# microsoft/YOLaT-VectorGraphicsRecognition

Measured on AMD Instinct MI355X. Metric: graphs_per_sec, higher is better.
Workload: dtype f32

## Files before the change

### include/yolat_hip.h

```cpp
#ifndef YOLAT_HIP_H
#define YOLAT_HIP_H

#include <stddef.h>
#include <stdint.h>

#ifdef __cplusplus
extern "C" {
#endif

typedef void* yolat_stream_t;

#define YOLAT_E_INVALID   (-1)
#define YOLAT_E_UNSUPPORTED (-2)

#define YOLAT_STATUS_EDGE_RANGE  1
#define YOLAT_STATUS_SEG_UNSORTED 2
#define YOLAT_STATUS_SEG_RANGE   4
#define YOLAT_STATUS_NOT_LOCAL   8


int yolat_abi_version(void);
const char* yolat_strerror(int code);


size_t yolat_csr_work_elems(int64_t N, int64_t E);
int yolat_coo_to_csr(const int64_t* edge, int64_t stride_e, int64_t stride_c, int64_t E, int64_t N,
                     int32_t* row_ptr, int32_t* perm, int32_t* src_csr, int32_t* dst_csr,
                     int32_t* work, int32_t* status, yolat_stream_t stream);

size_t yolat_csc_work_elems(int64_t N);
int yolat_csc_by_source(const int32_t* src_csr, int64_t E, int64_t N, int32_t* col_ptr,
                        int32_t* slots, int32_t* work, yolat_stream_t stream);

int yolat_expand_ranges(const int32_t* start, const int32_t* prefix, int64_t S, int64_t total, int32_t* out,
                        yolat_stream_t stream);
size_t yolat_subgraph_work_elems(int64_t N, int64_t n_sub);
int yolat_subgraph_reindex(const int32_t* node_ids, int64_t n_sub, int64_t N, const int64_t* edge,
                           int64_t stride_e, int64_t stride_c, const int32_t* edge_ids, int64_t m_sub,
                           const int64_t* bbox_idx, int64_t* edge_out, int64_t* bbox_idx_out, int32_t* work,
                           int32_t* status, yolat_stream_t stream);
int yolat_gather_rows_bytes(const void* src, int64_t src_row_bytes, const int32_t* idx, int64_t rows,
                            int64_t row_bytes, void* dst, int64_t dst_row_bytes, yolat_stream_t stream);

int yolat_fixup_offsets(int64_t* edge, int64_t E, const int64_t* edge_ptr, int64_t* bbox_idx, int64_t N,
                        const int64_t* node_ptr, const int64_t* node_off, const int64_t* prop_off, int64_t B,
                        yolat_stream_t stream);

int yolat_segment_ptr(const int64_t* bbox_idx, int64_t N, int64_t P, int32_t* seg_ptr,
                      int32_t* node_seg, int32_t* status, yolat_stream_t stream);

size_t yolat_graph_work_elems(int64_t N, int64_t E);
int yolat_graph_prepare(const int64_t* edge, int64_t stride_e, int64_t stride_c, const float* e_attr,
                        const int64_t* bbox_idx, int64_t E, int64_t N, int64_t P, int32_t* row_ptr,
                        int32_t* perm, int32_t* src_csr, int32_t* dst_csr, float* attr_csr,
                        int32_t* seg_ptr, int32_t* node_seg, int32_t* work, int32_t* status,
                        yolat_stream_t stream);

int yolat_graph_prepare_plan(int64_t N, int64_t E, int64_t other_wgs, int32_t* rows, int32_t* csr_wgs);

int yolat_gather_rows(const float* src, int64_t ld_src, const int32_t* idx, int64_t rows,
                      int64_t width, float* dst, int64_t ld_dst, yolat_stream_t stream);


#define YOLAT_STATS_ROWS 32
size_t yolat_bn_stats_elems(int64_t M, int64_t C);
int yolat_linear_fwd(const float* A, int64_t lda, int64_t M, int64_t K,
                     const float* a_scale, const float* a_shift, int a_relu,
                     const float* W, int64_t ldw, const float* bias, int64_t Nout,
                     const float* o_scale, const float* o_shift, int o_relu,
                     float* Y, int64_t ldy, int accumulate, float* stats, yolat_stream_t stream);

int yolat_linear_sk_x6(const float* A, int64_t lda, int64_t M, int64_t K, const float* W, int64_t ldw, const float* bias,
                       int64_t Nout, const float* o_scale, const float* o_shift, int o_relu, float* Y, int64_t ldy,
                       yolat_stream_t stream);

int yolat_linear_segmax_fwd(const float* A, int64_t lda, int64_t M, int64_t K, const float* W,
                            int64_t ldw, const float* bias, int64_t Nout, const float* o_scale,
                            const float* o_shift, const int32_t* node_seg, float* pool, int64_t ldpool,
                            yolat_stream_t stream);

int yolat_linear_fwd_wt(const float* A, int64_t lda, int64_t M, int64_t K,
                        const float* Wt, int64_t ldw, int64_t Nout,
                        float* Y, int64_t ldy, int accumulate, yolat_stream_t stream);

size_t yolat_linear_bwd_w_work_elems(int64_t M, int64_t Nout, int64_t K);
int yolat_linear_bwd_w(const float* dY, int64_t lddy, int64_t M, int64_t Nout,
                       const float* A, int64_t lda, int64_t K,
                       const float* a_scale, const float* a_shift, int a_relu,
                       float* dW, int64_t lddw, float* db, int accumulate,
                       float* partial, yolat_stream_t stream);

int yolat_bn_finalize(const float* stats, int64_t M, int64_t C, const float* gamma,
                      const float* beta, float* running_mean, float* running_var,
                      float momentum, float eps, float* save_mean, float* save_invstd,
                      float* scale, float* shift, yolat_stream_t stream);

int yolat_bn_eval_coeffs(const float* gamma, const float* beta, const float* running_mean,
                         const float* running_var, float eps, int64_t C, float* scale,
                         float* shift, yolat_stream_t stream);

int yolat_scale_shift_relu(const float* Y, int64_t ldy, int64_t M, int64_t C, const float* scale,
                           const float* shift, int relu, float* Z, int64_t ldz,
                           yolat_stream_t stream);

size_t yolat_bn_bwd_work_elems(int64_t M, int64_t C);
int yolat_bn_relu_bwd(const float* dZ, int64_t lddz, const float* Y, int64_t ldy, int64_t M,
                      int64_t C, const float* gamma, const float* save_mean,
                      const float* save_invstd, const float* scale, const float* shift, int relu,
                      float* dgamma, float* dbeta, int accumulate, float* dY, int64_t lddy,
                      float* work, yolat_stream_t stream);


int yolat_edge_lin1_fwd(const float* x, int64_t ldx, int64_t N, int64_t Cin,
                        const int32_t* src_csr, const int32_t* dst_csr, const float* attr_csr,
                        int64_t E, const float* W1, int64_t ldw, const float* b1, int64_t C,
                        const float* o_scale, const float* o_shift, int o_relu,
                        float* H1, int64_t ldh, float* stats, yolat_stream_t stream);

int yolat_edge_lin1_bwd_w(const float* dH1, int64_t lddh, int64_t E, int64_t C,
                          const float* x, int64_t ldx, int64_t N, int64_t Cin,
                          const int32_t* src_csr, const int32_t* dst_csr, const float* attr_csr,
                          float* dW1, int64_t lddw, float* db1, int accumulate, float* partial,
                          yolat_stream_t stream);

int yolat_edge_lin1_bwd_x(const float* dH1, int64_t lddh, int64_t E, int64_t C, const float* W1,
                          int64_t ldw, int64_t Cin, float* dG, int64_t lddg,
                          yolat_stream_t stream);

int yolat_edge_scatter_bwd(const float* dG, int64_t lddg, int64_t Cin, const int32_t* row_ptr,
                           const int32_t* col_ptr, const int32_t* slots, int64_t N, float* dX,
                           int64_t lddx, int accumulate, yolat_stream_t stream);

int yolat_edge_mlp2_eval(const float* x, int64_t ldx, int64_t N, int64_t Cin, const int32_t* src_csr,
                         const int32_t* dst_csr, const float* attr_csr, int64_t E, const float* W1,
                         const float* b1, const float* s1, const float* t1, const float* W2,
                         const float* b2, const float* s2, const float* t2, int64_t C, float* H2,
                         int64_t ldh, yolat_stream_t stream);

int yolat_graph_prepare_node_uv(const int64_t* edge, int64_t stride_e, int64_t stride_c, const float* e_attr,
                                const int64_t* bbox_idx, int64_t E, int64_t N, int64_t P, int32_t* row_ptr,
                                int32_t* perm, int32_t* src_csr, int32_t* dst_csr, float* attr_csr,
                                int32_t* seg_ptr, int32_t* node_seg, int32_t* work, int32_t* status, const float* x,
                                int64_t ldx, int64_t Cin, const float* Wuv, const float* uv_bias, const float* Wr,
                                const float* br,
                                const float* Wn, const float* bn, const float* sn, const float* tn, int64_t C,
                                float* UV, int64_t ld_uv, float* f_out, int64_t ld_fo, float* s_out, int64_t ld_so,
                                yolat_stream_t stream);

int yolat_conv_split_w1(const float* W1, int64_t Cin, int64_t C, float* Wuv, float* Wc4, yolat_stream_t stream);
int yolat_node_uv_eval(const float* f_in, int64_t ld_f, const float* s_in, int64_t ld_s, int64_t N, int64_t Cin,
                       const float* Wuv, const float* uv_bias, const float* Wr, const float* br, const float* Wn,
                       const float* bn, const float* sn, const float* tn, int64_t C, float* UV, int64_t ld_uv,
                       float* f_out, int64_t ld_fo, float* s_out, int64_t ld_so, yolat_stream_t stream);
int yolat_edge_uv_lin1_fwd(const float* UV, int64_t ld_uv, const int32_t* src_csr, const int32_t* dst_csr,
                           const float* attr_csr, int64_t E, const float* Wc4, const float* b1, int64_t C,
                           float* H1, int64_t ldh, float* stats, yolat_stream_t stream);

int yolat_edge_uv_sums(const float* dH1, int64_t ldh, const int32_t* row_ptr, const int32_t* col_ptr,
                       const int32_t* slots, int64_t N, int64_t C, float* dUV, int64_t ld_uv, yolat_stream_t stream);
int yolat_conv_merge_dw1(const float* dWuv, const float* dWc4, int64_t Cin, int64_t C, float* dW1, int64_t lddw,
                         int accumulate, yolat_stream_t stream);

#define YOLAT_EDGE_AUTO 0
#define YOLAT_EDGE_TILES 1
#define YOLAT_EDGE_WS_F32 2
#define YOLAT_EDGE_WS_X6 3
int yolat_edge_uv_mlp2_mean_eval(const float* UV, int64_t ld_uv, const int32_t* src_csr, const int32_t* dst_csr,
                                 const float* attr_csr, const int32_t* row_ptr, int64_t N, int64_t E,
                                 const float* Wc4, const float* b1, const float* s1, const float* t1,
                                 const float* W2, const float* b2, const float* s2, const float* t2, int64_t C,
                                 float* f_out, int64_t ld_fo, yolat_stream_t stream);
int yolat_edge_uv_mlp2_mean_eval_variant(const float* UV, int64_t ld_uv, const int32_t* src_csr,
                                         const int32_t* dst_csr, const float* attr_csr, const int32_t* row_ptr,
                                         int64_t N, int64_t E, const float* Wc4, const float* b1, const float* s1,
                                         const float* t1, const float* W2, const float* b2, const float* s2,
                                         const float* t2, int64_t C, float* f_out, int64_t ld_fo, int variant,
                                         yolat_stream_t stream);
int yolat_edge_uv_mlp2_eval(const float* UV, int64_t ld_uv, const int32_t* src_csr, const int32_t* dst_csr,
                            const float* attr_csr, int64_t E, const float* Wc4, const float* b1, const float* s1,
                            const float* t1, const float* W2, const float* b2, const float* s2, const float* t2,
                            int64_t C, float* H2, int64_t ldh, yolat_stream_t stream);

int yolat_node_side_eval(const float* f_in, int64_t ld_f, const float* s_in, int64_t ld_s, int64_t N,
                         int64_t Cin, const float* Wr, const float* br, const float* Wn, const float* bn,
                         const float* sn, const float* tn, const float* H2, int64_t ldh,
                         const int32_t* row_ptr, int64_t E, int64_t C, float* f_out, int64_t ld_fo,
                         float* s_out, int64_t ld_so, yolat_stream_t stream);

int yolat_csr_mean_fwd(const float* H, int64_t ldh, int64_t C, const float* h_scale,
                       const float* h_shift, int h_relu, const int32_t* row_ptr, int64_t N,
                       float* out, int64_t ldo, int accumulate, yolat_stream_t stream);

int yolat_csr_mean_bwd(const float* dOut, int64_t lddo, int64_t C, const int32_t* row_ptr,
                       const int32_t* dst_csr, int64_t E, float* dM, int64_t lddm,
                       yolat_stream_t stream);

int yolat_segment_mean_fwd(const float* X, int64_t ldx, int64_t D, const float* x_scale,
                           const float* x_shift, int x_relu, const int32_t* seg_ptr, int64_t P,
                           float* Y, int64_t ldy, yolat_stream_t stream);
int yolat_segment_max_fwd(const float* X, int64_t ldx, int64_t D, const float* x_scale,
                          const float* x_shift, int x_relu, const int32_t* seg_ptr, int64_t P,
                          int64_t N, float* Y, int64_t ldy, int32_t* arg ,
                          yolat_stream_t stream);
int yolat_fusion_pair_eval(const float* A, int64_t lda, int64_t N, int64_t D, const float* Wf, const float* bf,
                           const float* sf, const float* tf, int64_t F, const int32_t* node_seg, float* pool,
                           int64_t ldpool, const float* S, int64_t lds, int64_t P, const float* Wfs,
                           const float* bfs, const float* sfs, const float* tfs, float* Ys, int64_t ldys,
                           yolat_stream_t stream);

int yolat_pool_prepare(const float* feats, const float* fsup, int64_t ld, int64_t D, int64_t F,
                       const int32_t* seg_ptr, int64_t P, float* Z, int64_t ldz, yolat_stream_t stream);

int yolat_segment_mean_bwd(const float* dY, int64_t lddy, int64_t D, const int32_t* seg_ptr,
                           const int32_t* node_seg, int64_t N, float* dX, int64_t lddx,
                           yolat_stream_t stream);
int yolat_segment_max_bwd(const float* dY, int64_t lddy, int64_t D, const int32_t* arg,
                          const int32_t* node_seg, int64_t N, float* dX, int64_t lddx,
                          yolat_stream_t stream);

size_t yolat_fusion_pool_train_saved_elems(int64_t K, int64_t F, int64_t P);
size_t yolat_fusion_pool_train_work_elems(int64_t N, int64_t K, int64_t F, int64_t P);
int yolat_fusion_pool_train_fwd(const float* A, int64_t lda, int64_t N, int64_t K, const float* W,
                                const float* bias, int64_t F, const float* gamma, const float* beta,
                                float* running_mean, float* running_var, float momentum, float eps,
                                const int32_t* node_seg, int64_t P, float* Z, int64_t ldz, float* coef,
                                float* saved, float* work, yolat_stream_t stream);
int yolat_fusion_pool_train_bwd(const float* A, int64_t lda, int64_t N, int64_t K, const float* W,
                                const float* gamma, int64_t F, const float* coef, const float* saved,
                                const int32_t* node_seg, const int32_t* seg_ptr, int64_t P, const float* gZ,
                                int64_t ldg, float* dW, float* dbias, float* dgamma, float* dbeta, float* dA,
                                int64_t ldda, float* work, yolat_stream_t stream);
#define YOLAT_FUS_BWD_COLS 1
#define YOLAT_FUS_BWD_DW 2
#define YOLAT_FUS_BWD_DA 4
#define YOLAT_FUS_BWD_ALL 7
int yolat_fusion_pool_train_bwd_parts(const float* A, int64_t lda, int64_t N, int64_t K, const float* W,
                                      const float* gamma, int64_t F, const float* coef, const float* saved,
                                      const int32_t* node_seg, const int32_t* seg_ptr, int64_t P, const float* gZ,
                                      int64_t ldg, float* dW, float* dbias, float* dgamma, float* dbeta, float* dA,
                                      int64_t ldda, float* work, int parts, yolat_stream_t stream);


size_t yolat_softmax_ce_work_elems(int64_t P);
int yolat_softmax_ce(const float* logits, int64_t ld, const int64_t* labels, int64_t P, int64_t K,
                     float* loss, float* dlogits, int64_t lddl, float* work, yolat_stream_t stream);

int yolat_sigmoid(const float* z, int64_t ldz, int64_t P, int64_t K, float* out, int64_t ldo, yolat_stream_t stream);
int yolat_sigmoid_bwd(const float* dp, int64_t lddp, const float* p, int64_t ldp, int64_t P, int64_t K, float* dz,
                      int64_t lddz, yolat_stream_t stream);
size_t yolat_bce_work_elems(int64_t P);
int yolat_bce(const float* prob, int64_t ld, const int64_t* labels, int64_t P, int64_t K, float* loss, float* dprob,
              int64_t lddp, float* work, yolat_stream_t stream);
int yolat_sigmoid_bce(const float* logits, int64_t ld, const int64_t* labels, int64_t P, int64_t K, float* loss,
                      float* dlogits, int64_t lddl, float* prob, int64_t ldp, float* work, yolat_stream_t stream);

int yolat_adam_step(float* param, const float* grad, float* exp_avg, float* exp_avg_sq, int64_t n,
                    float lr, float beta1, float beta2, float eps, float weight_decay,
                    int64_t step, float grad_scale, yolat_stream_t stream);

#define YOLAT_MAX_LAYERS 8

typedef struct {
  int64_t Cin;
  const float *W1, *b1, *s1, *t1;
  const float *W2, *b2, *s2, *t2;
  const float *Wr, *br;
  const float *Wn, *bn, *sn, *tn;
  const float *Wuv, *Wc4;
  const float *Wuvf, *uvb, *Wc4f, *t2f;
  const uint16_t *Wfr_x6[3];
  const float *tfr;
  const uint16_t *Wn_x6[3];
  const float *tn_fold;
  const float *Wnx, *tnx;
} yolat_conv_eval;

#define YOLAT_CLS_X6_MAX_ROWS 2048
#define YOLAT_CLS1_X6_MIN_ROWS 1024
#define YOLAT_NODE_X6_MIN_ROWS 65536
typedef struct {
  int32_t n_blocks, n_blocks_out, n_classes, reserved;
  int64_t C;
  int64_t F;
  int64_t H1, H2;
  yolat_conv_eval conv[YOLAT_MAX_LAYERS];
  const float *Wf, *bf, *sf, *tf;
  const uint16_t *Wf_hi, *Wf_mid, *Wf_lo;
  const float *tf_fold;
  const uint16_t *Wfs_hi, *Wfs_mid, *Wfs_lo;
  const float *tfs_fold;
  const float *Wfs, *bfs, *sfs, *tfs;
  const float *Wc1, *bc1, *sc1, *tc1;
  const float *Wc2, *bc2, *sc2, *tc2;
  const float *Wc3, *bc3;
  const uint16_t *Wc_x6[3];
  const float *tc_fold[3];
  const uint16_t *Wc1_gx;
  const float *tc1_gx;
} yolat_model_eval;

size_t yolat_forward_eval_workspace_bytes(const yolat_model_eval* m, int64_t N, int64_t E, int64_t P);

int yolat_forward_eval(const yolat_model_eval* m, const float* x, int64_t ldx, const int64_t* edge,
                       int64_t stride_e, int64_t stride_c, const float* e_attr,
                       const int64_t* bbox_idx, int64_t N, int64_t E, int64_t P, float* logits,
                       int64_t ld_logits, void* workspace, size_t workspace_bytes, int32_t* status,
                       yolat_stream_t stream);
int yolat_forward_eval_primed(const yolat_model_eval* m, const float* x, int64_t ldx, const int64_t* edge,
                              int64_t stride_e, int64_t stride_c, const float* e_attr,
                              const int64_t* bbox_idx, int64_t N, int64_t E, int64_t P, float* logits,
                              int64_t ld_logits, void* workspace, size_t workspace_bytes, int32_t* status,
                              yolat_stream_t stream);

typedef struct { const void* ptr; int64_t bytes; } yolat_span;
int yolat_collate_pack(void* dst, const int64_t* field_off, const yolat_span* spans, int64_t n_fields, int64_t n_items);
int yolat_item_csr_host(const int64_t* edge, int64_t stride_e, int64_t stride_c, const float* e_attr,
                        const int64_t* bbox_idx, int64_t E, int64_t N, int64_t P, int32_t* row_ptr, int32_t* perm,
                        int32_t* src, int32_t* dst, float* attr, int32_t* seg_ptr, int32_t* node_seg, int32_t* status);
typedef struct {
  int64_t N, E, P;
  const int32_t *row_ptr, *src, *dst;
  const float* attr;
  const int32_t *seg_ptr, *node_seg;
} yolat_item_csr;
int yolat_collate_csr_pack(const yolat_item_csr* items, int64_t B, int32_t* row_ptr, int32_t* src, int32_t* dst,
                           float* attr, int32_t* seg_ptr, int32_t* node_seg);

#define YOLAT_MAX_KEYS 8
typedef struct {
  int64_t n_keys;
  yolat_span key[YOLAT_MAX_KEYS];
  int64_t rows[YOLAT_MAX_KEYS];
  yolat_item_csr csr;
  int32_t fix[YOLAT_MAX_KEYS];
  int32_t node_key, prop_key;
} yolat_item_desc;
int yolat_collate_batch(const yolat_item_desc* const* items, int64_t B, void* dst, int64_t cap, int64_t* off,
                        int64_t* total, int64_t* slices, int64_t* totals);

typedef struct yolat_loader yolat_loader;
typedef struct {
  void* device;
  int64_t total, n_keys, B, N, E, P;
  int64_t off[YOLAT_MAX_KEYS + 6];
  const int64_t* slices;
  int32_t slot, rc;
} yolat_loader_batch;
yolat_loader* yolat_loader_create(int slots);
int yolat_loader_submit(yolat_loader* loader, const yolat_item_desc* const* items, int64_t B);
int yolat_loader_next(yolat_loader* loader, yolat_stream_t consumer_stream, yolat_loader_batch* out);
int yolat_loader_release(yolat_loader* loader, int slot, yolat_stream_t consumer_stream);
void yolat_loader_destroy(yolat_loader* loader);

typedef struct {
  const int32_t *row_ptr, *src, *dst;
  const float* attr;
  const int32_t *seg_ptr, *node_seg;
} yolat_graph_csr;
int yolat_forward_eval_csr(const yolat_model_eval* m, const float* x, int64_t ldx, const yolat_graph_csr* g, int64_t N,
                           int64_t E, int64_t P, float* logits, int64_t ld_logits, void* workspace,
                           size_t workspace_bytes, yolat_stream_t stream);

typedef struct {
  const yolat_model_eval* base;
  const uint16_t* Wuv[YOLAT_MAX_LAYERS];
  const uint16_t* Wr[YOLAT_MAX_LAYERS];
  const uint16_t* Wn[YOLAT_MAX_LAYERS];
  const uint16_t* W2[YOLAT_MAX_LAYERS];
  const float* uv_scale[YOLAT_MAX_LAYERS];
  const float* uv_shift[YOLAT_MAX_LAYERS];
  const uint16_t *Wf, *Wfs, *Wc1, *Wc2, *Wc3;
  const float* t2f[YOLAT_MAX_LAYERS];
  const uint16_t *Wf_fold, *Wfs_fold;
  const float *tf_fold, *tfs_fold;
  const void* conv_local;
} yolat_model_eval_bf16;

size_t yolat_conv_local_pack_bytes(int64_t n_layers);
int yolat_conv_local_pack(const yolat_model_eval_bf16* m, void* dst, size_t dst_bytes, yolat_stream_t stream);
void yolat_conv_local_tune(int nw, int g0, int abl, long long* stamps);
int yolat_conv_stack_local_bf16(const yolat_model_eval_bf16* m, const void* pack, const float* x, int64_t ldx,
                                const yolat_graph_csr* g, int64_t N, int64_t E, int64_t P, uint16_t* feats,
                                int64_t ld_feats, float* Z, int64_t ldz, int32_t* flag, yolat_stream_t stream);

#define YOLAT_LOC_UNGROUPED 1
#define YOLAT_LOC_CROSSING  2
#define YOLAT_LOC_MALFORMED 4
typedef struct yolat_locality {
  int32_t known, flags, max_nodes, max_edges;
} yolat_locality;
size_t yolat_batch_locality_workspace_bytes(int64_t N, int64_t E, int64_t P);
int yolat_batch_locality(const int64_t* edge, int64_t stride_e, int64_t stride_c, const int64_t* bbox_idx, int64_t N,
                         int64_t E, int64_t P, int32_t* info, void* workspace, size_t workspace_bytes,
                         yolat_stream_t stream);
int yolat_conv_local_fits(const yolat_locality* loc, int64_t P);
// ... 248 lines not shown
```

### yolat_vectorgraphicsrecognition_amd/_lib.py

```python
import ctypes
import os

_HERE = os.path.dirname(os.path.abspath(__file__))
LIB_PATH = os.environ.get("YOLAT_LIB_PATH") or os.path.join(_HERE, "libyolat_hip.so")

c_p = ctypes.c_void_p
c_i64 = ctypes.c_int64
c_int = ctypes.c_int
c_f = ctypes.c_float
c_sz = ctypes.c_size_t

YOLAT_MAX_LAYERS = 8


class ConvEval(ctypes.Structure):
    _fields_ = ([("Cin", c_i64)] + [(n, c_p) for n in
                                    ("W1", "b1", "s1", "t1", "W2", "b2", "s2", "t2", "Wr", "br", "Wn", "bn", "sn", "tn",
                                     "Wuv", "Wc4", "Wuvf", "uvb", "Wc4f", "t2f")] +
                [("Wfr_x6", c_p * 3), ("tfr", c_p), ("Wn_x6", c_p * 3), ("tn_fold", c_p), ("Wnx", c_p), ("tnx", c_p)])


class ModelEval(ctypes.Structure):
    _fields_ = ([("n_blocks", ctypes.c_int32), ("n_blocks_out", ctypes.c_int32), ("n_classes", ctypes.c_int32),
                 ("reserved", ctypes.c_int32), ("C", c_i64), ("F", c_i64), ("H1", c_i64), ("H2", c_i64),
# ... 42 lines not shown


class Locality(ctypes.Structure):
    _fields_ = [("known", ctypes.c_int32), ("flags", ctypes.c_int32), ("max_nodes", ctypes.c_int32),
                ("max_edges", ctypes.c_int32)]


class TrainLin(ctypes.Structure):
    _fields_ = [("W", c_p), ("b", c_p)]


class TrainBn(ctypes.Structure):
    _fields_ = [("gamma", c_p), ("beta", c_p), ("running_mean", c_p), ("running_var", c_p), ("num_batches_tracked", c_p),
                ("momentum", c_f), ("eps", c_f)]


class TrainConv(ctypes.Structure):
    _fields_ = [("Cin", c_i64), ("nn0", TrainLin), ("bn1", TrainBn), ("nn3", TrainLin), ("bn4", TrainBn), ("lin_r", TrainLin),
                ("node", TrainLin), ("bn_node", TrainBn)]


class TrainModel(ctypes.Structure):
    _fields_ = [("n_blocks", ctypes.c_int32), ("n_blocks_out", ctypes.c_int32), ("n_classes", ctypes.c_int32),
                ("half", ctypes.c_int32), ("C", c_i64), ("F", c_i64), ("H1", c_i64), ("H2", c_i64),
                ("conv", TrainConv * YOLAT_MAX_LAYERS), ("fus", TrainLin), ("fus_bn", TrainBn), ("fus_s", TrainLin),
                ("fus_s_bn", TrainBn), ("c1", TrainLin), ("c1_bn", TrainBn), ("c2", TrainLin), ("c2_bn", TrainBn),
                ("c3", TrainLin), ("param_base", c_p), ("grad_base", c_p)]


class AdamArgs(ctypes.Structure):
    _fields_ = [("exp_avg", c_p), ("exp_avg_sq", c_p), ("n", c_i64), ("step", c_i64), ("lr", c_f), ("beta1", c_f),
                ("beta2", c_f), ("eps", c_f), ("weight_decay", c_f), ("grad_scale", c_f)]


class PredictTree(ctypes.Structure):
    _fields_ = [("R", c_i64), ("Ctot", c_i64), ("B", c_i64), ("root_row", c_p), ("root_range", c_p), ("child_ptr", c_p),
                ("child_row", c_p), ("child_range", c_p), ("image_root_ptr", c_p)]


class GraphCsr(ctypes.Structure):
    _fields_ = [("row_ptr", c_p), ("src", c_p), ("dst", c_p), ("attr", c_p), ("seg_ptr", c_p), ("node_seg", c_p)]


SIGNATURES = {
    "yolat_abi_version": (c_int, []),
    "yolat_strerror": (ctypes.c_char_p, [c_int]),
    "yolat_csr_work_elems": (c_sz, [c_i64, c_i64]),
    "yolat_coo_to_csr": (c_int, [c_p, c_i64, c_i64, c_i64, c_i64, c_p, c_p, c_p, c_p, c_p, c_p, c_p]),
    "yolat_edge_mlp2_eval": (c_int, [c_p, c_i64, c_i64, c_i64, c_p, c_p, c_p, c_i64, c_p, c_p, c_p, c_p, c_p, c_p, c_p,
                                      c_p, c_i64, c_p, c_i64, c_p]),
    "yolat_node_side_eval": (c_int, [c_p, c_i64, c_p, c_i64, c_i64, c_i64, c_p, c_p, c_p, c_p, c_p, c_p, c_p, c_i64,
                                      c_p, c_i64, c_i64, c_p, c_i64, c_p, c_i64, c_p]),
    "yolat_fusion_pool_train_saved_elems": (c_sz, [c_i64, c_i64, c_i64]),
    "yolat_fusion_pool_train_work_elems": (c_sz, [c_i64, c_i64, c_i64, c_i64]),
    "yolat_fusion_pool_train_fwd": (c_int, [c_p, c_i64, c_i64, c_i64, c_p, c_p, c_i64, c_p, c_p, c_p, c_p, c_f, c_f,
                                             c_p, c_i64, c_p, c_i64, c_p, c_p, c_p, c_p]),
    "yolat_fusion_pool_train_bwd": (c_int, [c_p, c_i64, c_i64, c_i64, c_p, c_p, c_i64, c_p, c_p, c_p, c_p, c_i64, c_p,
                                             c_i64, c_p, c_p, c_p, c_p, c_p, c_i64, c_p, c_p]),
    "yolat_fusion_pool_train_bwd_parts": (c_int, [c_p, c_i64, c_i64, c_i64, c_p, c_p, c_i64, c_p, c_p, c_p, c_p, c_i64, c_p,
                                                   c_i64, c_p, c_p, c_p, c_p, c_p, c_i64, c_p, c_int, c_p]),
    "yolat_fusion_pool_train_fwd_bf16": (c_int, [c_p, c_i64, c_i64, c_i64, c_p, c_p, c_i64, c_p, c_p, c_p, c_p, c_f, c_f,
                                                  c_p, c_i64, c_p, c_i64, c_p, c_p, c_p, c_p]),
    "yolat_fusion_pool_train_bwd_parts_bf16": (c_int, [c_p, c_i64, c_i64, c_i64, c_p, c_p, c_i64, c_p, c_p, c_p, c_p, c_i64,
                                                        c_p, c_i64, c_p, c_p, c_p, c_p, c_p, c_i64, c_p, c_int, c_p]),
    "yolat_bt_linear_fwd": (c_int, [c_p, c_i64, c_i64, c_i64, c_p, c_p, c_int, c_p, c_i64, c_p, c_i64, c_p, c_i64, c_p, c_p]),
    "yolat_bt_linear_fwd_wt": (c_int, [c_p, c_i64, c_i64, c_i64, c_p, c_i64, c_i64, c_p, c_i64, c_int, c_p]),
    "yolat_bt_linear_bwd_w_work_elems": (c_sz, [c_i64, c_i64, c_i64]),
    "yolat_bt_linear_bwd_w": (c_int, [c_p, c_i64, c_i64, c_i64, c_p, c_i64, c_i64, c_p, c_p, c_int, c_p, c_i64, c_p, c_p,
                                       c_p]),
    "yolat_expand_ranges": (c_int, [c_p, c_p, c_i64, c_i64, c_p, c_p]),
    "yolat_subgraph_work_elems": (c_sz, [c_i64, c_i64]),
    "yolat_subgraph_reindex": (c_int, [c_p, c_i64, c_i64, c_p, c_i64, c_i64, c_p, c_i64, c_p, c_p, c_p, c_p, c_p, c_p]),
    "yolat_gather_rows_bytes": (c_int, [c_p, c_i64, c_p, c_i64, c_i64, c_p, c_i64, c_p]),
    "yolat_fixup_offsets": (c_int, [c_p, c_i64, c_p, c_p, c_i64, c_p, c_p, c_p, c_i64, c_p]),
    "yolat_conv_split_w1": (c_int, [c_p, c_i64, c_i64, c_p, c_p, c_p]),
    "yolat_node_uv_eval": (c_int, [c_p, c_i64, c_p, c_i64, c_i64, c_i64, c_p, c_p, c_p, c_p, c_p, c_p, c_p, c_p, c_i64,
                                    c_p, c_i64, c_p, c_i64, c_p, c_i64, c_p]),
    "yolat_edge_uv_mlp2_eval": (c_int, [c_p, c_i64, c_p, c_p, c_p, c_i64, c_p, c_p, c_p, c_p, c_p, c_p, c_p, c_p, c_i64,
                                         c_p, c_i64, c_p]),
    "yolat_edge_uv_mlp2_mean_eval": (c_int, [c_p, c_i64, c_p, c_p, c_p, c_p, c_i64, c_i64, c_p, c_p, c_p, c_p, c_p, c_p,
                                              c_p, c_p, c_i64, c_p, c_i64, c_p]),
    "yolat_edge_uv_mlp2_mean_eval_variant": (c_int, [c_p, c_i64, c_p, c_p, c_p, c_p, c_i64, c_i64, c_p, c_p, c_p, c_p,
                                                      c_p, c_p, c_p, c_p, c_i64, c_p, c_i64, c_int, c_p]),
    "yolat_edge_uv_sums": (c_int, [c_p, c_i64, c_p, c_p, c_p, c_i64, c_i64, c_p, c_i64, c_p]),
    "yolat_conv_merge_dw1": (c_int, [c_p, c_p, c_i64, c_i64, c_p, c_i64, c_int, c_p]),
    "yolat_fusion_pair_eval": (c_int, [c_p, c_i64, c_i64, c_i64, c_p, c_p, c_p, c_p, c_i64, c_p, c_p, c_i64, c_p, c_i64,
                                        c_i64, c_p, c_p, c_p, c_p, c_p, c_i64, c_p]),
    "yolat_graph_prepare_node_uv": (c_int, [c_p, c_i64, c_i64, c_p, c_p, c_i64, c_i64, c_i64] + [c_p] * 9 +
                                    [c_p, c_i64, c_i64] + [c_p] * 8 + [c_i64, c_p, c_i64, c_p, c_i64, c_p, c_i64, c_p]),
    "yolat_csc_work_elems": (c_sz, [c_i64]),
    "yolat_csc_by_source": (c_int, [c_p, c_i64, c_i64, c_p, c_p, c_p, c_p]),
    "yolat_segment_ptr": (c_int, [c_p, c_i64, c_i64, c_p, c_p, c_p, c_p]),
    "yolat_graph_work_elems": (c_sz, [c_i64, c_i64]),
    "yolat_graph_prepare": (c_int, [c_p, c_i64, c_i64, c_p, c_p, c_i64, c_i64, c_i64, c_p, c_p, c_p, c_p, c_p,
                                    c_p, c_p, c_p, c_p, c_p]),
    "yolat_graph_prepare_plan": (c_int, [c_i64, c_i64, c_i64, c_p, c_p]),
    "yolat_gather_rows": (c_int, [c_p, c_i64, c_p, c_i64, c_i64, c_p, c_i64, c_p]),
    "yolat_bn_stats_elems": (c_sz, [c_i64, c_i64]),
    "yolat_linear_fwd": (c_int, [c_p, c_i64, c_i64, c_i64, c_p, c_p, c_int,
                                 c_p, c_i64, c_p, c_i64, c_p, c_p, c_int,
                                 c_p, c_i64, c_int, c_p, c_p]),
    "yolat_linear_sk_x6": (c_int, [c_p, c_i64, c_i64, c_i64, c_p, c_i64, c_p, c_i64, c_p, c_p, c_int, c_p, c_i64, c_p]),
    "yolat_linear_segmax_fwd": (c_int, [c_p, c_i64, c_i64, c_i64, c_p, c_i64, c_p, c_i64, c_p, c_p, c_p, c_p, c_i64,
                                        c_p]),
    "yolat_linear_fwd_wt": (c_int, [c_p, c_i64, c_i64, c_i64, c_p, c_i64, c_i64, c_p, c_i64, c_int, c_p]),
    "yolat_linear_bwd_w_work_elems": (c_sz, [c_i64, c_i64, c_i64]),
    "yolat_linear_bwd_w": (c_int, [c_p, c_i64, c_i64, c_i64, c_p, c_i64, c_i64, c_p, c_p, c_int,
                                   c_p, c_i64, c_p, c_int, c_p, c_p]),
    "yolat_bn_finalize": (c_int, [c_p, c_i64, c_i64, c_p, c_p, c_p, c_p, c_f, c_f, c_p, c_p, c_p, c_p, c_p]),
    "yolat_bn_eval_coeffs": (c_int, [c_p, c_p, c_p, c_p, c_f, c_i64, c_p, c_p, c_p]),
    "yolat_scale_shift_relu": (c_int, [c_p, c_i64, c_i64, c_i64, c_p, c_p, c_int, c_p, c_i64, c_p]),
    "yolat_bn_bwd_work_elems": (c_sz, [c_i64, c_i64]),
    "yolat_bn_relu_bwd": (c_int, [c_p, c_i64, c_p, c_i64, c_i64, c_i64, c_p, c_p, c_p, c_p, c_p, c_int,
                                  c_p, c_p, c_int, c_p, c_i64, c_p, c_p]),
    "yolat_edge_lin1_fwd": (c_int, [c_p, c_i64, c_i64, c_i64, c_p, c_p, c_p, c_i64, c_p, c_i64, c_p,
                                    c_i64, c_p, c_p, c_int, c_p, c_i64, c_p, c_p]),
    "yolat_edge_lin1_bwd_w": (c_int, [c_p, c_i64, c_i64, c_i64, c_p, c_i64, c_i64, c_i64, c_p, c_p, c_p,
                                      c_p, c_i64, c_p, c_int, c_p, c_p]),
    "yolat_edge_lin1_bwd_x": (c_int, [c_p, c_i64, c_i64, c_i64, c_p, c_i64, c_i64, c_p, c_i64, c_p]),
    "yolat_edge_scatter_bwd": (c_int, [c_p, c_i64, c_i64, c_p, c_p, c_p, c_i64, c_p, c_i64, c_int, c_p]),
    "yolat_csr_mean_fwd": (c_int, [c_p, c_i64, c_i64, c_p, c_p, c_int, c_p, c_i64, c_p, c_i64, c_int, c_p]),
    "yolat_csr_mean_bwd": (c_int, [c_p, c_i64, c_i64, c_p, c_p, c_i64, c_p, c_i64, c_p]),
    "yolat_segment_mean_fwd": (c_int, [c_p, c_i64, c_i64, c_p, c_p, c_int, c_p, c_i64, c_p, c_i64, c_p]),
    "yolat_segment_max_fwd": (c_int, [c_p, c_i64, c_i64, c_p, c_p, c_int, c_p, c_i64, c_i64, c_p, c_i64,
                                      c_p, c_p]),
    "yolat_pool_prepare": (c_int, [c_p, c_p, c_i64, c_i64, c_i64, c_p, c_i64, c_p, c_i64, c_p]),
    "yolat_segment_mean_bwd": (c_int, [c_p, c_i64, c_i64, c_p, c_p, c_i64, c_p, c_i64, c_p]),
    "yolat_segment_max_bwd": (c_int, [c_p, c_i64, c_i64, c_p, c_p, c_i64, c_p, c_i64, c_p]),
    "yolat_softmax_ce_work_elems": (c_sz, [c_i64]),
    "yolat_softmax_ce": (c_int, [c_p, c_i64, c_p, c_i64, c_i64, c_p, c_p, c_i64, c_p, c_p]),
    "yolat_sigmoid": (c_int, [c_p, c_i64, c_i64, c_i64, c_p, c_i64, c_p]),
    "yolat_sigmoid_bwd": (c_int, [c_p, c_i64, c_p, c_i64, c_i64, c_i64, c_p, c_i64, c_p]),
    "yolat_bce_work_elems": (c_sz, [c_i64]),
    "yolat_bce": (c_int, [c_p, c_i64, c_p, c_i64, c_i64, c_p, c_p, c_i64, c_p, c_p]),
    "yolat_sigmoid_bce": (c_int, [c_p, c_i64, c_p, c_i64, c_i64, c_p, c_p, c_i64, c_p, c_i64, c_p, c_p]),
    "yolat_adam_step": (c_int, [c_p, c_p, c_p, c_p, c_i64, c_f, c_f, c_f, c_f, c_f, c_i64, c_f, c_p]),
    "yolat_profile_enabled": (c_int, []),
    "yolat_profile_enable": (c_int, [c_int]),
    "yolat_profile_reset": (c_int, []),
    "yolat_profile_count": (c_int, []),
    "yolat_profile_get": (c_int, [c_int, ctypes.c_char_p, c_int, ctypes.POINTER(c_f), ctypes.POINTER(c_int),
                                  ctypes.POINTER(ctypes.c_double), ctypes.POINTER(ctypes.c_double)]),
    "yolat_forward_eval_workspace_bytes": (c_sz, [ctypes.POINTER(ModelEval), c_i64, c_i64, c_i64]),
    "yolat_forward_eval": (c_int, [ctypes.POINTER(ModelEval), c_p, c_i64, c_p, c_i64, c_i64, c_p, c_p, c_i64, c_i64,
                                   c_i64, c_p, c_i64, c_p, c_sz, c_p, c_p]),
    "yolat_forward_eval_primed": (c_int, [ctypes.POINTER(ModelEval), c_p, c_i64, c_p, c_i64, c_i64, c_p, c_p, c_i64,
                                          c_i64, c_i64, c_p, c_i64, c_p, c_sz, c_p, c_p]),
    "yolat_edge_uv_lin1_fwd": (c_int, [c_p, c_i64, c_p, c_p, c_p, c_i64, c_p, c_p, c_i64, c_p, c_i64, c_p, c_p]),
    "yolat_nms_work_bytes": (c_sz, [c_i64]),
    "yolat_nms": (c_int, [c_p, c_p, c_i64, c_f, c_p, c_p, c_p, c_sz, c_p]),
    "yolat_detect_scores": (c_int, [c_p, c_i64, c_i64, c_i64, c_p, c_p, c_i64, c_p, c_int, c_p, c_p]),
    "yolat_nms_batched_work_bytes": (c_sz, [c_i64, c_i64, c_i64]),
    "yolat_nms_batched": (c_int, [c_p, c_i64, c_i64, c_p, c_i64, c_f, c_f, c_int, c_p, c_p, c_p, c_sz, c_p]),
    "yolat_detect_match": (c_int, [c_p, c_p, c_i64, c_p, c_p, c_i64, c_p, c_p, c_i64, c_p, c_p]),
    "yolat_f32_to_bf16": (c_int, [c_p, c_i64, c_p, c_p]),
    "yolat_edge_uv_lin1_fwd_h": (c_int, [c_p, c_i64, c_p, c_p, c_p, c_i64, c_p, c_p, c_i64, c_p, c_i64, c_p, c_p]),
    "yolat_linear_fwd_h": (c_int, [c_p, c_i64, c_i64, c_i64, c_p, c_p, c_int, c_p, c_i64, c_p, c_i64, c_p, c_i64, c_p,
                                   c_p, c_p]),
    "yolat_csr_mean_fwd_h": (c_int, [c_p, c_i64, c_i64, c_p, c_p, c_int, c_p, c_i64, c_p, c_i64, c_int, c_p]),
    "yolat_csr_mean_bwd_h": (c_int, [c_p, c_i64, c_i64, c_p, c_p, c_i64, c_p, c_i64, c_p]),
    "yolat_bn_relu_bwd_h": (c_int, [c_p, c_i64, c_p, c_i64, c_i64, c_i64, c_p, c_p, c_p, c_p, c_int, c_p, c_p, c_int,
                                    c_p, c_i64, c_p, c_p]),
    "yolat_linear_bwd_w_h": (c_int, [c_p, c_i64, c_i64, c_i64, c_p, c_int, c_i64, c_i64, c_p, c_p, c_int, c_p, c_i64,
                                     c_p, c_int, c_p, c_p]),
    "yolat_linear_fwd_wt_h": (c_int, [c_p, c_i64, c_i64, c_i64, c_p, c_i64, c_i64, c_p, c_i64, c_p, c_p]),
    "yolat_edge_uv_sums_h": (c_int, [c_p, c_i64, c_p, c_p, c_p, c_i64, c_i64, c_p, c_i64, c_p]),
    "yolat_split_bf16x3": (c_int, [c_p, c_i64, c_i64, c_i64, c_p, c_p, c_p, c_p, c_p]),
    "yolat_linear_fwd_rows_x6": (c_int, [c_p, c_i64, c_i64, c_i64, c_p, c_p, c_int, c_p, c_i64, c_p, c_i64, c_p, c_i64, c_p,
                                         c_p, c_p]),
    "yolat_node_uv_eval_x6": (c_int, [c_p, c_i64, c_p, c_i64, c_i64, c_p, c_p, c_p, c_p, c_p, c_p, c_p, c_p, c_p, c_i64,
                                      c_p, c_i64, c_p, c_i64, c_p]),
    "yolat_fusion_pair_eval_x6": (c_int, [c_p, c_i64, c_i64, c_i64, c_p, c_p, c_p, c_p, c_i64, c_p, c_p, c_i64, c_p,
                                          c_i64, c_i64, c_p, c_p, c_p, c_p, c_p, c_i64, c_p]),
    "yolat_inv_degree": (c_int, [c_p, c_i64, c_p, c_p]),
    "yolat_bn_csr_work_elems": (c_sz, [c_i64, c_i64]),
    "yolat_bn_csr_bwd_stats": (c_int, [ctypes.POINTER(BnCsrGrad), c_i64, c_i64, c_p, c_p, c_int, c_p, c_p, c_p]),
    "yolat_linear_bwd_w_csr": (c_int, [ctypes.POINTER(BnCsrGrad), c_i64, c_i64, c_p, c_i64, c_i64, c_p, c_p, c_int, c_p,
                                       c_i64, c_p, c_int, c_p, c_p]),
    "yolat_linear_fwd_wt_csr": (c_int, [ctypes.POINTER(BnCsrGrad), c_i64, c_i64, c_p, c_i64, c_i64, c_p, c_i64, c_p]),
# ... 107 lines not shown
```

### yolat_vectorgraphicsrecognition_amd/csrc/common.hpp

```cpp
#pragma once
#include <hip/hip_runtime.h>
#include <stdint.h>

#include "../../include/yolat_hip.h"

typedef float f32x16 __attribute__((ext_vector_type(16)));
typedef float f32x4 __attribute__((ext_vector_type(4)));

#define YL_LAUNCH_CHECK()                          \
  do {                                             \
    hipError_t e__ = hipGetLastError();            \
    if (e__ != hipSuccess) return (int)e__;        \
  } while (0)

#define YL_TRY(call)            \
  do {                          \
    int rc__ = (call);          \
    if (rc__ != 0) return rc__; \
  } while (0)

static inline int yl_cdiv(long a, long b) { return (int)((a + b - 1) / b); }
static inline bool yl_aligned16(const void* p) { return (((uintptr_t)p) & 15) == 0; }

struct Carver {
// ... 694 lines not shown
#pragma unroll
        for (int k = 0; k < N3_KMAX; ++k) acc = fmaf(x[k], w[j][k], acc);
        v[j] = fmaxf(fmaf(acc + b[j], sc[j], sh[j]), floor);
      }
      const int row = rb + u;
      if (row < r1) {
        if (Yh != nullptr) {
          uint2 o;
          o.x = yl_pack_bf16(v[0], v[1]); o.y = yl_pack_bf16(v[2], v[3]);
          *reinterpret_cast<uint2*>(Yh + (long)row * ldy + col) = o;
        } else {
          *reinterpret_cast<float4*>(Y + (long)row * ldy + col) = make_float4(v[0], v[1], v[2], v[3]);
        }
      }
    }
  }
}

bool yl_node3_smallk_ok(const NodeUv& a);
bool yl_node3_smallk_shape_ok(const NodeUv& a);
int yl_node3_smallk(const NodeUv& a, hipStream_t st, YlGate gate = YlGate{nullptr, 0});
int yl_fusion_rows_x6_key64(const float* A, long lda, long N, long K, const float* W, const float* bias, long F,
                            const float* sgn, const int* node_seg, unsigned long long* keys, uint16_t* wsplit,
                            yolat_stream_t stream);
int yl_fusion_rows_bf16_key64(const float* A, long lda, long N, long K, const float* W, const float* bias, long F,
                              const float* sgn, const int* node_seg, unsigned long long* keys, uint16_t* wimg,
                              yolat_stream_t stream);
#define YL_POOL_ZERO 1
#define YL_POOL_MAX 2
#define YL_POOL_MEAN 4
struct PoolRider {
  const float* feats; const float* fsup; long ld; int D, F, P; const int* seg_ptr; float* Z; long ldz;
  int parts, blocks;
};
__device__ __forceinline__ void yl_pool_rider(const PoolRider& r, int vb, int nvb, int tid, int nthreads) {
  const int wz = (r.parts & YL_POOL_ZERO) ? r.F : 0, wx = (r.parts & YL_POOL_MAX) ? r.D : 0,
            wm = (r.parts & YL_POOL_MEAN) ? r.D : 0;
  const int W = wz + wx + wm;
  const long total = (long)r.P * W;
  for (long i = (long)vb * nthreads + tid; i < total; i += (long)nvb * nthreads) {
    const int p = (int)(i / W), c = (int)(i - (long)p * W);
    float* z = r.Z + (long)p * r.ldz;
    if (c < wz) { z[c] = 0.f; continue; }
    const bool is_max = c < wz + wx;
    const int k = is_max ? c - wz : c - wz - wx;
    const float* src = (is_max ? r.feats : r.fsup) + k;
    const int r0 = r.seg_ptr[p], r1 = r.seg_ptr[p + 1];
    float best = 0.f, sm = 0.f;
    bool any = false;
    int q = r0;
    for (; q + 8 <= r1; q += 8) {
      float v[8];
#pragma unroll
      for (int j = 0; j < 8; ++j) v[j] = src[(long)(q + j) * r.ld];
#pragma unroll
      for (int j = 0; j < 8; ++j) {
        if (!any || v[j] > best) { best = v[j]; any = true; }
        sm += v[j];
      }
    }
    for (; q < r1; ++q) {
      const float v = src[(long)q * r.ld];
      if (!any || v > best) { best = v; any = true; }
      sm += v;
    }
    if (is_max) z[r.F + k] = best;
    else {
      const int cnt = r1 - r0;
      z[2 * r.F + r.D + k] = sm / (float)(cnt > 1 ? cnt : 1);
    }
  }
}
struct EdgeNext {
  const float* Wp; const float* bias; float* UV; long ld_uv; float* root; long ld_root;
  const float* s_in; long ld_si; const float* Wn; const float* bn; const float* sn; const float* tn;
  float* s_out; long ld_so; int s_tiles;
};
int yl_edge_tile_groups(int64_t N, int64_t E);
int yl_edge_uv_mlp2_mean_eval_impl(const float* UV, int64_t ld_uv, const int32_t* src_csr, const int32_t* dst_csr,
                                   const float* attr_csr, const int32_t* row_ptr, int64_t N, int64_t E, const float* Wc4,
                                   const float* b1, const float* s1, const float* t1, const float* W2, const float* b2,
                                   const float* s2, const float* t2, int64_t C, float* f_out, int64_t ld_fo, int variant,
                                   const PoolRider* rider, int* rode, const EdgeNext* next, int* did_next,
                                   yolat_stream_t stream);
int yl_fusion_pair_eval_x6_impl(const float* A, int64_t lda, int64_t N, int64_t D, const uint16_t* Wh, const uint16_t* Wm,
                                const uint16_t* Wl, const float* tfold, int64_t F, const int32_t* node_seg, float* pool,
                                int64_t ldpool, const float* S, int64_t lds, int64_t P, const uint16_t* Wsh,
                                const uint16_t* Wsm, const uint16_t* Wsl, const float* tsfold, float* Ys, int64_t ldys,
                                const PoolRider* rider, yolat_stream_t stream);
int yl_pool_prepare_parts(const float* feats, const float* fsup, int64_t ld, int64_t D, int64_t F, const int32_t* seg_ptr,
                          int64_t P, float* Z, int64_t ldz, int parts, yolat_stream_t stream);
bool yl_profile_on();
void yl_stage_begin(const char* name, double flops, double bytes, yolat_stream_t stream);
void yl_stage_end(yolat_stream_t stream);

struct YlLocalIn {
  const int32_t *row_ptr, *src, *dst; const float* attr; const int32_t* seg_ptr;
  const int64_t* edge; int64_t se, sc; const int32_t* eptr;
  int32_t* status;
};
int yl_local_prep(const int64_t* edge, int64_t se, int64_t sc, const int64_t* bbox_idx, int64_t N, int64_t E, int64_t P,
                  int32_t* seg_ptr, int32_t* node_seg, int32_t* eptr, int32_t* status, int32_t* info, bool vouched,
                  hipStream_t st);

int yl_graph_prepare_impl(const int64_t* edge, int64_t stride_e, int64_t stride_c, const float* e_attr,
                          const int64_t* bbox_idx, int64_t E, int64_t N, int64_t P, int32_t* row_ptr, int32_t* perm,
                          int32_t* src_csr, int32_t* dst_csr, float* attr_csr, int32_t* seg_ptr, int32_t* node_seg,
                          int32_t* work, int32_t* status, const NodeUv* extra, bool primed, yolat_stream_t stream);
template <int BK>
__device__ __forceinline__ void node_uv_tile(const NodeUv& a, int x, int y) {
  if (y < 2) gemm_nt_tile<64, 64, BK, DenseOp, DenseOp, false>(a.af, a.wuv, a.euv, a.N, 2 * a.C, a.Cin, x, y);
  else if (y == 2) gemm_nt_tile<64, 64, BK, DenseOp, DenseOp, false>(a.af, a.wr, a.er, a.N, a.C, a.Cin, x, 0);
  else gemm_nt_tile<64, 64, BK, DenseOp, DenseOp, false>(a.as, a.wn, a.en, a.N, a.C, a.Cin, x, 0);
}

template <int BK>
__global__ void __launch_bounds__(256) k_gemm_nt_node3(NodeUv a) {
  node_uv_tile<BK>(a, blockIdx.x, blockIdx.y);
}

template <class AL, class BL, bool B_NFAST>
__global__ void __launch_bounds__(256) k_gemm_nt_sk(AL A, BL B, Epilogue ep, int M, int N, int K) {
  constexpr int BT = 32, BK = 128, LD = BK + 1;
  __shared__ float smem[2 * BT * LD];
  float* As = smem;
  float* Bs = smem + BT * LD;
  const int tid = threadIdx.x, wave = tid >> 6, lane = tid & 63;
  const int l31 = lane & 31, lhi = lane >> 5;
  int rt_, ct_;
  yl_xcd_tile(rt_, ct_);
  const int row0 = rt_ * BT, col0 = ct_ * BT;
  const bool fastA = A.vec != 0, fastB = B.vec != 0;
  auto map_r = [](int i) { return 4 * ((i >> 5) & 7) + ((i & 31) >> 3); };
  auto map_q = [](int i) { return 8 * (i >> 8) + (i & 7); };
  const EpiPre pre = epi_prefetch(ep, row0, col0 + l31, M, N);

  f32x16 acc;
#pragma unroll
  for (int r = 0; r < 16; ++r) acc[r] = 0.f;

  float ra0[4][4], rb0[4][4], ra1[4][4], rb1[4][4];
  auto fetch = [&](int k0, float (&ra)[4][4], float (&rb)[4][4]) {
    const bool full = (k0 + BK <= K);
    if (full && fastA) {
#pragma unroll
      for (int t = 0; t < 4; ++t) {
        const int i = tid + t * 256;
        A.template load4<true>(row0 + map_r(i), k0 + 4 * map_q(i), ra[t]);
      }
    } else {
#pragma unroll
      for (int t = 0; t < 4; ++t) {
        const int i = tid + t * 256;
        A.template load4<false>(row0 + map_r(i), k0 + 4 * map_q(i), ra[t]);
      }
    }
    if (full && fastB) {
#pragma unroll
      for (int t = 0; t < 4; ++t) {
        const int i = tid + t * 256;
        const int n = B_NFAST ? (i % BT) : map_r(i);
        const int kq = B_NFAST ? (i / BT) : map_q(i);
        B.template load4<true>(col0 + n, k0 + 4 * kq, rb[t]);
      }
    } else {
#pragma unroll
      for (int t = 0; t < 4; ++t) {
        const int i = tid + t * 256;
        const int n = B_NFAST ? (i % BT) : map_r(i);
        const int kq = B_NFAST ? (i / BT) : map_q(i);
        B.template load4<false>(col0 + n, k0 + 4 * kq, rb[t]);
      }
    }
  };
  auto stage = [&](float (&ra)[4][4], float (&rb)[4][4]) {
#pragma unroll
    for (int t = 0; t < 4; ++t) {
      const int i = tid + t * 256;
      float* d = As + map_r(i) * LD + 4 * map_q(i);
      d[0] = ra[t][0]; d[1] = ra[t][1]; d[2] = ra[t][2]; d[3] = ra[t][3];
      const int n = B_NFAST ? (i % BT) : map_r(i);
      const int kq = B_NFAST ? (i / BT) : map_q(i);
      float* e = Bs + n * LD + 4 * kq;
      e[0] = rb[t][0]; e[1] = rb[t][1]; e[2] = rb[t][2]; e[3] = rb[t][3];
    }
  };
  auto compute = [&]() {
    const int kb = wave * 32;
#pragma unroll
    for (int kk = 0; kk < 32; kk += 2) {
      const float a = As[l31 * LD + kb + kk + lhi];
// ... 321 lines not shown
```

### yolat_vectorgraphicsrecognition_amd/csrc/edge.hip

```cpp
#include "common.hpp"
#include <stdlib.h>

extern "C" int yolat_edge_lin1_fwd(const float* x, int64_t ldx, int64_t N, int64_t Cin,
                                   const int32_t* src_csr, const int32_t* dst_csr,
                                   const float* attr_csr, int64_t E, const float* W1, int64_t ldw,
                                   const float* b1, int64_t C, const float* o_scale,
                                   const float* o_shift, int o_relu, float* H1, int64_t ldh,
                                   float* stats, yolat_stream_t stream) {
  if (E < 0 || N <= 0 || Cin <= 0 || C <= 0 || !x || !W1) return YOLAT_E_INVALID;
  if (E == 0) return 0;
  if (!src_csr || !dst_csr || !attr_csr || !H1 || E >= (1LL << 31)) return YOLAT_E_INVALID;
  const long K = 2 * Cin + 4;
  if (ldw < K || ldh < C || ldx < Cin) return YOLAT_E_INVALID;
  if ((o_scale == nullptr) != (o_shift == nullptr)) return YOLAT_E_INVALID;
  EdgeOp a = yl_edge(x, ldx, Cin, src_csr, dst_csr, attr_csr, E);
  DenseOp b = yl_dense(W1, ldw, C, K);
  Epilogue ep;
  ep.bias = b1; ep.scale = o_scale; ep.shift = o_shift; ep.relu = o_relu;
  ep.Y = H1; ep.ldy = ldh; ep.accumulate = 0; ep.stats = stats; ep.seg = nullptr; ep.pool = nullptr; ep.ldpool = 0;
  hipStream_t st = (hipStream_t)stream;
  dim3 grid(yl_cdiv(E, 64), yl_cdiv(C, 64));
  if (K <= 16)
    hipLaunchKernelGGL((k_gemm_nt<64, 64, 16, EdgeOp, DenseOp, false>), grid, dim3(256), 0, st, a,
                       b, ep, (int)E, (int)C, (int)K);
// ... 361 lines not shown
#pragma unroll 8
    for (int kk = 0; kk < 64; kk += 2) {
      const float av = Hs[(wm * 32 + l31) * LDH + kk + lhi];
      const float bv = W2s[(wn * 32 + l31) * LDH + kk + lhi];
      acc2 = __builtin_amdgcn_mfma_f32_32x32x2f32(av, bv, acc2, 0, 0, 0);
    }
    if (c0 == e0) EDGE_STAMP(5);
    __syncthreads();
#pragma unroll
    for (int r = 0; r < 16; ++r) {
      const int row = wm * 32 + (r & 3) + 8 * (r >> 2) + 4 * lhi;
      Hs[row * LDH + col] = fmaxf(fmaf(acc2[r] + bias2, sc2, sh2), 0.f);
    }
    __syncthreads();
    if (c0 == e0) EDGE_STAMP(6);
#pragma unroll
    for (int j = 0; j < NG; ++j) {
      if (rb + 16 * j < nn) {
        const int lo = my_b[j] > c0 ? my_b[j] : c0;
        const int hi = my_e[j] < c0 + 64 ? my_e[j] : c0 + 64;
        for (int e = lo; e < hi; ++e) {
          const float* m = Hs + (e - c0) * LDH + 4 * q;
          sum[j].x += m[0]; sum[j].y += m[1]; sum[j].z += m[2]; sum[j].w += m[3];
        }
      }
    }
    if (c0 == e0) EDGE_STAMP(7);
    __syncthreads();
  }
  EDGE_STAMP(8);
#pragma unroll
  for (int j = 0; j < NG; ++j) {
    const int deg = my_e[j] - my_b[j];
    if (rb + 16 * j < nn && deg > 0) {
      const float inv = 1.f / (float)deg;
      float4* o = reinterpret_cast<float4*>(f_out + (long)(n0 + rb + 16 * j) * ld_fo + 4 * q);
      float4 d = fo[j];
      d.x = yl_mul_rn(sum[j].x, inv) + d.x; d.y = yl_mul_rn(sum[j].y, inv) + d.y;
      d.z = yl_mul_rn(sum[j].z, inv) + d.z; d.w = yl_mul_rn(sum[j].w, inv) + d.w;
      *o = d;
      fo[j] = d;
    }
  }
  EDGE_STAMP(9);
  if constexpr (NG == 1 && NEXT) {
    float bfa[16], bfb[16];
#pragma unroll
    for (int ks = 0; ks < 16; ++ks) bfa[ks] = nx.Wp[(wave * 16 + ks) * 64 + lane];
    float* frow = Hs + rb * LDH + 4 * q;
    const float4 fz = (rb < nn) ? fo[0] : make_float4(0.f, 0.f, 0.f, 0.f);
    frow[0] = fz.x; frow[1] = fz.y; frow[2] = fz.z; frow[3] = fz.w;
    __syncthreads();
    const int fr = lane & 15, fk = lane >> 4;
#pragma unroll
    for (int t = 0; t < 3; ++t) {
      const int ct = wave + 4 * t;
      if (t < 2) {
#pragma unroll
        for (int ks = 0; ks < 16; ++ks) bfb[ks] = nx.Wp[((ct + 4) * 16 + ks) * 64 + lane];
      }
      const int col = ct * 16 + fr;
      const float bias = nx.bias[col];
      f32x4 acc = {0.f, 0.f, 0.f, 0.f};
#pragma unroll
      for (int ks = 0; ks < 16; ++ks)
        acc = __builtin_amdgcn_mfma_f32_16x16x4f32(Hs[fr * LDH + 4 * ks + fk], bfa[ks], acc, 0, 0, 0);
#pragma unroll
      for (int r = 0; r < 4; ++r) {
        const int row = 4 * fk + r;
        if (row < nn) {
          const float v = acc[r] + bias;
          if (col < 128) nx.UV[(long)(n0 + row) * nx.ld_uv + col] = v;
          else nx.root[(long)(n0 + row) * nx.ld_root + (col - 128)] = v;
        }
      }
#pragma unroll
      for (int ks = 0; ks < 16; ++ks) bfa[ks] = bfb[ks];
    }
  }
  EDGE_STAMP(10);
#ifdef YOLAT_EDGE_STAMPS
  if (threadIdx.x == 0 && blockIdx.x < 4096) edge_stamps_d[nx.Wp != nullptr ? 0 : 1][blockIdx.x * 16 + 11] = (long long)((e1g - e0g + 63) / 64);
#endif
}

typedef __bf16 yl_bf16x8 __attribute__((ext_vector_type(8)));
typedef unsigned yl_u32x4 __attribute__((ext_vector_type(4)));
__device__ __forceinline__ void yl_split8(const float x[8], yl_bf16x8& h, yl_bf16x8& m, yl_bf16x8& l) {
  yl_u32x4 ph, pm, pl;
#pragma unroll
  for (int i = 0; i < 4; ++i) {
    const unsigned x0 = __float_as_uint(x[2 * i]), x1 = __float_as_uint(x[2 * i + 1]);
    const yl_f32x2 xv = {x[2 * i], x[2 * i + 1]};
    const yl_f32x2 hv = {__uint_as_float(x0 & 0xffff0000u), __uint_as_float(x1 & 0xffff0000u)};
    const yl_f32x2 hmv = {__uint_as_float(x0 & 0xffffff00u), __uint_as_float(x1 & 0xffffff00u)};
    const yl_f32x2 mv = hmv - hv, lv = xv - hmv;
    ph[i] = __builtin_amdgcn_perm(x1, x0, 0x07060302u);
    pm[i] = __builtin_amdgcn_perm(__float_as_uint(mv.y), __float_as_uint(mv.x), 0x07060302u);
    pl[i] = __builtin_amdgcn_perm(__float_as_uint(lv.y), __float_as_uint(lv.x), 0x07060302u);
  }
  h = *reinterpret_cast<yl_bf16x8*>(&ph);
  m = *reinterpret_cast<yl_bf16x8*>(&pm);
  l = *reinterpret_cast<yl_bf16x8*>(&pl);
}

template <bool FOLD, bool X6>
__global__ void __launch_bounds__(512, 4) k_edge_uv_mlp2_mean_ws(const float* __restrict__ UV, long ld_uv,
                                                                 const int* __restrict__ src,
                                                                 const int* __restrict__ dst,
                                                                 const float* __restrict__ attr,
                                                                 const int* __restrict__ row_ptr, int N, int E, int chunk,
                                                                 const float* __restrict__ Wc4,
                                                                 const float* __restrict__ b1,
                                                                 const float* __restrict__ s1,
                                                                 const float* __restrict__ t1,
                                                                 const float* __restrict__ W2,
                                                                 const float* __restrict__ b2,
                                                                 const float* __restrict__ s2,
                                                                 const float* __restrict__ t2, float* f_out, long ld_fo) {
  constexpr int LDH = 68, TILE = 64 * LDH;
  __shared__ __attribute__((aligned(16))) float Hs[2 * TILE];
  __shared__ __attribute__((aligned(16))) float Ms[2 * TILE];
  __shared__ int seg_start[2][66];
  __shared__ int seg_node[2][64];
  __shared__ int seg_info[2][4];
  __shared__ __attribute__((aligned(16))) float carry_s[2][64];
  __shared__ int carry_cnt_s[2];
  const int tid = threadIdx.x, wave = tid >> 6, lane = tid & 63;
  const long c_lo = (long)blockIdx.x * chunk;
  if (c_lo >= E) return;
  const long c_hi = c_lo + chunk;
  int eS = 0, eE = E;
  if (c_lo > 0) {
    const int n = dst[c_lo];
    eS = (row_ptr[n] == (int)c_lo) ? (int)c_lo : row_ptr[n + 1];
  }
  if (c_hi < E) {
    const int n = dst[c_hi];
    eE = (row_ptr[n] == (int)c_hi) ? (int)c_hi : row_ptr[n + 1];
  }
  if (eS >= eE) return;
  const int np = (eE - eS + 63) >> 6;

  if (wave >= 4) {
    const int cw = wave - 4, wm = cw >> 1, wn = cw & 1, l31 = lane & 31, lhi = lane >> 5;
    const int col = wn * 32 + l31;
    const float bias2 = (!FOLD && b2) ? b2[col] : 0.f, sc2 = s2 ? s2[col] : 1.f, sh2 = s2 ? t2[col] : 0.f;
    auto store_messages = [&](const f32x16& acc, int p) {
      float* ms = Ms + (p & 1) * TILE;
#pragma unroll
      for (int r = 0; r < 16; ++r) {
        const int row = wm * 32 + (r & 3) + 8 * (r >> 2) + 4 * lhi;
        ms[row * LDH + col] = FOLD ? fmaxf(fmaf(acc[r], sc2, sh2), 0.f) : fmaxf(fmaf(acc[r] + bias2, sc2, sh2), 0.f);
      }
    };
    if (X6) {
      yl_bf16x8 Bh[4], Bm[4], Bl[4];
#pragma unroll
      for (int ks = 0; ks < 4; ++ks) {
        const float4* wp = reinterpret_cast<const float4*>(W2 + (long)col * 64 + 16 * ks + 8 * lhi);
        const float4 w0 = wp[0], w1 = wp[1];
        float x[8] = {w0.x, w0.y, w0.z, w0.w, w1.x, w1.y, w1.z, w1.w};
        if (FOLD) {
#pragma unroll
          for (int i = 0; i < 8; ++i) x[i] *= sc2;
        }
// ... 142 lines not shown
    }
    const int first_next = __shfl(dm_nxt, 0);
    if (lane == 63) seg_info[bsel][2] = (c0 + 64 < eE && first_next == dm_cur) ? 1 : 0;
    prev_last = __shfl(dm_cur, 63);
    dm_cur = dm_nxt;
    dm_nxt = dst[yl_min(c0 + 128 + lane, eE - 1)];
  };
  float4 fo0 = make_float4(0.f, 0.f, 0.f, 0.f);
  auto fo_load = [&](int P) {
    const int bsel = P & 1;
    const int k = yl_min(rb, seg_info[bsel][0] - 1);
    fo0 = *reinterpret_cast<const float4*>(f_out + (long)seg_node[bsel][k] * ld_fo + 4 * q);
  };
  auto aggregate = [&](int P) {
    const int bsel = P & 1;
    const float* ms = Ms + bsel * TILE + 4 * q;
    const int nseg = seg_info[bsel][0], cont_in = seg_info[bsel][1], cont_out = seg_info[bsel][2];
    for (int k = rb; k < nseg; k += 16) {
      const int lo = seg_start[bsel][k], hi = seg_start[bsel][k + 1];
      float4 sm = make_float4(0.f, 0.f, 0.f, 0.f);
      int cn = 0;
      if (k == 0 && cont_in) {
        sm = *reinterpret_cast<const float4*>(&carry_s[bsel ^ 1][4 * q]);
        cn = carry_cnt_s[bsel ^ 1];
      }
      for (int r = lo; r < hi; ++r) {
        const float4 m = *reinterpret_cast<const float4*>(ms + r * LDH);
        sm.x += m.x; sm.y += m.y; sm.z += m.z; sm.w += m.w;
      }
      cn += hi - lo;
      if (k == nseg - 1 && cont_out) {
        *reinterpret_cast<float4*>(&carry_s[bsel][4 * q]) = sm;
        if (q == 0) carry_cnt_s[bsel] = cn;
      } else {
        const float inv = 1.f / (float)cn;
        float4* o = reinterpret_cast<float4*>(f_out + (long)seg_node[bsel][k] * ld_fo + 4 * q);
        float4 d = fo0;
        if (k != rb) d = *o;
        d.x = yl_mul_rn(sm.x, inv) + d.x; d.y = yl_mul_rn(sm.y, inv) + d.y;
        d.z = yl_mul_rn(sm.z, inv) + d.z; d.w = yl_mul_rn(sm.w, inv) + d.w;
        *o = d;
      }
    }
  };
  load_idx(eS);
  gather(eS);
  load_idx(eS + 64);
  layer1(Hs);
  gather(eS + 64);
  load_idx(eS + 128);
  __syncthreads();
  for (int p = 0; p < np; ++p) {
    layer1(Hs + ((p + 1) & 1) * TILE);
    gather(eS + 64 * (p + 2));
    load_idx(eS + 64 * (p + 3));
    meta(p);
    if (p >= 1) aggregate(p - 1);
    fo_load(p);
    __syncthreads();
  }
  aggregate(np - 1);
}

static long edge_tile_npt(long N, long E) {
  long npt = (56 * N) / E;
  const long npt2 = (112 * N) / E < 16 ? (112 * N) / E : 16;
  if (npt2 >= 2 * npt - 2 && N / (npt2 > 0 ? npt2 : 1) >= 8192) npt = npt2;
  if (npt < 1) npt = 1;
  if (npt > 64) npt = 64;
  return npt;
}
int yl_edge_tile_groups(int64_t N, int64_t E) {
  if (N <= 0 || E <= 0) return 0;
  const int variant = E >= 131072 ? (yl_strict_fp32() ? YOLAT_EDGE_WS_F32 : YOLAT_EDGE_WS_X6) : YOLAT_EDGE_TILES;
  if (variant != YOLAT_EDGE_TILES) return 0;
  return edge_tile_npt(N, E) <= 16 ? 1 : 4;
}

int yl_edge_uv_mlp2_mean_eval_impl(const float* UV, int64_t ld_uv, const int32_t* src_csr, const int32_t* dst_csr,
                                   const float* attr_csr, const int32_t* row_ptr, int64_t N, int64_t E, const float* Wc4,
                                   const float* b1, const float* s1, const float* t1, const float* W2, const float* b2,
                                   const float* s2, const float* t2, int64_t C, float* f_out, int64_t ld_fo, int variant,
                                   const PoolRider* rider, int* rode, const EdgeNext* next, int* did_next,
                                   yolat_stream_t stream) {
  if (rode) *rode = 0;
  if (did_next) *did_next = 0;
  if (E < 0 || N <= 0 || !UV || !Wc4 || !W2 || !row_ptr || !f_out) return YOLAT_E_INVALID;
  if (variant < YOLAT_EDGE_AUTO || variant > YOLAT_EDGE_WS_X6) return YOLAT_E_INVALID;
  if (C != 64) return YOLAT_E_UNSUPPORTED;
  if (E == 0) return 0;
  if (!src_csr || !dst_csr || !attr_csr || E >= (1LL << 31) || ld_fo < C || ld_uv < 2 * C) return YOLAT_E_INVALID;
  if ((s1 == nullptr) != (t1 == nullptr) || (s2 == nullptr) != (t2 == nullptr)) return YOLAT_E_INVALID;
  if (ld_uv % 4 != 0 || ld_fo % 4 != 0 || !yl_aligned16(UV) || !yl_aligned16(attr_csr) || !yl_aligned16(Wc4) ||
      (b1 && !yl_aligned16(b1)) || !yl_aligned16(f_out) || (s1 && (!yl_aligned16(s1) || !yl_aligned16(t1))))
    return YOLAT_E_UNSUPPORTED;
  const bool fold = b1 == nullptr && s1 == nullptr && b2 == nullptr;
  const long ws_wgs = 512;
  const bool ws_ok = yl_aligned16(W2) && E >= 64 && N * ld_uv * 4 < (1LL << 32) && E * 16 < (1LL << 32);
  if (variant == YOLAT_EDGE_AUTO) {
    variant = E >= 131072 ? (yl_strict_fp32() ? YOLAT_EDGE_WS_F32 : YOLAT_EDGE_WS_X6) : YOLAT_EDGE_TILES;
    if (!ws_ok) variant = YOLAT_EDGE_TILES;
  } else if (variant != YOLAT_EDGE_TILES && !ws_ok) {
    return YOLAT_E_UNSUPPORTED;
  }
  if (variant != YOLAT_EDGE_TILES) {
    long chunk = ((E + ws_wgs - 1) / ws_wgs + 63) / 64 * 64;
    if (chunk < 64) chunk = 64;
    const unsigned grid = (unsigned)((E + chunk - 1) / chunk);
#define YL_WS_LAUNCH(F, X)                                                                                          \
  hipLaunchKernelGGL((k_edge_uv_mlp2_mean_ws<F, X>), dim3(grid), dim3(512), 0, (hipStream_t)stream, UV, (long)ld_uv,   \
                     src_csr, dst_csr, attr_csr, row_ptr, (int)N, (int)E, (int)chunk, Wc4, b1, s1, t1, W2, b2, s2, t2, \
                     f_out, (long)ld_fo)
    if (variant == YOLAT_EDGE_WS_X6) { if (fold) YL_WS_LAUNCH(true, true); else YL_WS_LAUNCH(false, true); }
    else { if (fold) YL_WS_LAUNCH(true, false); else YL_WS_LAUNCH(false, false); }
#undef YL_WS_LAUNCH
    YL_LAUNCH_CHECK();
    return 0;
  }
  const long npt = edge_tile_npt(N, E);
  DenseOp w2 = yl_dense(W2, C, C, C);
  const int tiles = yl_cdiv(N, npt);
  PoolRider pr{};
  if (rider && rider->blocks > 0) { pr = *rider; if (rode) *rode = 1; }
  EdgeNext nx{};
  if (next && next->Wp && npt <= 16) {
    if (!next->bias || !next->UV || !next->root || next->UV == UV) return YOLAT_E_INVALID;
    if (next->s_tiles > 0 && (!next->s_in || !next->Wn || !next->sn || !next->tn || !next->s_out || next->ld_si % 4 != 0 ||
                              !yl_aligned16(next->s_in) || !yl_aligned16(next->Wn)))
      return YOLAT_E_INVALID;
    nx = *next;
    if (did_next) *did_next = 1;
  }
  const unsigned grid = (unsigned)tiles + (unsigned)nx.s_tiles + (unsigned)pr.blocks;
  if (npt <= 16 && nx.Wp != nullptr)
    hipLaunchKernelGGL((k_edge_uv_mlp2_mean<1, true>), dim3(grid), dim3(256), 0, (hipStream_t)stream, UV, (long)ld_uv,
                       src_csr, dst_csr, attr_csr, row_ptr, (int)N, (int)npt, Wc4, b1, s1, t1, w2, b2, s2, t2, f_out,
                       (long)ld_fo, (int)E, tiles, pr, nx);
  else if (npt <= 16)
    hipLaunchKernelGGL((k_edge_uv_mlp2_mean<1, false>), dim3(grid), dim3(256), 0, (hipStream_t)stream, UV, (long)ld_uv,
                       src_csr, dst_csr, attr_csr, row_ptr, (int)N, (int)npt, Wc4, b1, s1, t1, w2, b2, s2, t2, f_out,
                       (long)ld_fo, (int)E, tiles, pr, nx);
  else
    hipLaunchKernelGGL((k_edge_uv_mlp2_mean<4, false>), dim3(grid), dim3(256), 0, (hipStream_t)stream, UV, (long)ld_uv,
                       src_csr, dst_csr, attr_csr, row_ptr, (int)N, (int)npt, Wc4, b1, s1, t1, w2, b2, s2, t2, f_out,
                       (long)ld_fo, (int)E, tiles, pr, nx);
  YL_LAUNCH_CHECK();
  return 0;
}

extern "C" int yolat_edge_uv_mlp2_mean_eval_variant(const float* UV, int64_t ld_uv, const int32_t* src_csr,
                                                    const int32_t* dst_csr, const float* attr_csr,
                                                    const int32_t* row_ptr, int64_t N, int64_t E, const float* Wc4,
                                                    const float* b1, const float* s1, const float* t1, const float* W2,
                                                    const float* b2, const float* s2, const float* t2, int64_t C,
                                                    float* f_out, int64_t ld_fo, int variant, yolat_stream_t stream) {
  return yl_edge_uv_mlp2_mean_eval_impl(UV, ld_uv, src_csr, dst_csr, attr_csr, row_ptr, N, E, Wc4, b1, s1, t1, W2, b2, s2,
                                        t2, C, f_out, ld_fo, variant, nullptr, nullptr, nullptr, nullptr, stream);
}

extern "C" int yolat_edge_uv_mlp2_mean_eval(const float* UV, int64_t ld_uv, const int32_t* src_csr,
                                            const int32_t* dst_csr, const float* attr_csr,
                                            const int32_t* row_ptr, int64_t N, int64_t E, const float* Wc4,
                                            const float* b1, const float* s1, const float* t1, const float* W2,
                                            const float* b2, const float* s2, const float* t2, int64_t C,
                                            float* f_out, int64_t ld_fo, yolat_stream_t stream) {
  return yolat_edge_uv_mlp2_mean_eval_variant(UV, ld_uv, src_csr, dst_csr, attr_csr, row_ptr, N, E, Wc4, b1, s1, t1, W2,
                                              b2, s2, t2, C, f_out, ld_fo, YOLAT_EDGE_AUTO, stream);
}

template <class TO>
__global__ void __launch_bounds__(256) k_edge_uv_lin1(const float* __restrict__ UV, long ld_uv,
                                                      const int* __restrict__ src, const int* __restrict__ dst,
                                                      const float* __restrict__ attr, int E,
                                                      const float* __restrict__ Wc4, const float* __restrict__ b1,
                                                      TO* __restrict__ H1, long ldh, float2* __restrict__ stats) {
  constexpr int LDT = 65;
  __shared__ float T[64 * LDT];
  const int tid = threadIdx.x, q = tid & 15, rb = tid >> 4;
  const int row0 = blockIdx.x * 64;
  float4 wc[4];
#pragma unroll
  for (int j = 0; j < 4; ++j) wc[j] = *reinterpret_cast<const float4*>(Wc4 + (4 * q + j) * 4);
  float4 bb = make_float4(0.f, 0.f, 0.f, 0.f);
  if (b1) bb = *reinterpret_cast<const float4*>(b1 + 4 * q);
  int di[4], si[4];
#pragma unroll
  for (int t = 0; t < 4; ++t) {
    const int e = yl_min(row0 + rb + 16 * t, E - 1);
    di[t] = dst[e]; si[t] = src[e];
  }
  float4 u[4], v[4], a[4];
#pragma unroll
  for (int t = 0; t < 4; ++t) {
    const int e = yl_min(row0 + rb + 16 * t, E - 1);
    u[t] = *reinterpret_cast<const float4*>(UV + (long)di[t] * ld_uv + 4 * q);
    v[t] = *reinterpret_cast<const float4*>(UV + (long)si[t] * ld_uv + 64 + 4 * q);
    a[t] = *reinterpret_cast<const float4*>(attr + (long)e * 4);
  }
#pragma unroll
  for (int t = 0; t < 4; ++t) {
    auto one = [&](float uu, float vv, const float4& w, float b) {
      float z = uu + vv;
      z = fmaf(a[t].x, w.x, z); z = fmaf(a[t].y, w.y, z); z = fmaf(a[t].z, w.z, z); z = fmaf(a[t].w, w.w, z);
      return z + b;
    };
    const float4 h = make_float4(one(u[t].x, v[t].x, wc[0], bb.x), one(u[t].y, v[t].y, wc[1], bb.y),
                                 one(u[t].z, v[t].z, wc[2], bb.z), one(u[t].w, v[t].w, wc[3], bb.w));
    const int r = rb + 16 * t;
    if (row0 + r < E) yl_st4(H1 + (long)(row0 + r) * ldh + 4 * q, h);
    float* tr = T + r * LDT + 4 * q;
    tr[0] = h.x; tr[1] = h.y; tr[2] = h.z; tr[3] = h.w;
  }
  if (stats == nullptr) return;
  __syncthreads();
  if (tid < 128) {
    const int c = tid & 63, grp = tid >> 6;
    const int base = row0 + 32 * grp;
    int cnt = E - base;
    cnt = cnt > 32 ? 32 : cnt;
    if (cnt == 32) {
      float v[32];
#pragma unroll
      for (int r = 0; r < 32; ++r) v[r] = T[(32 * grp + r) * LDT + c];
      float sum = 0.f;
#pragma unroll
      for (int r = 0; r < 32; ++r) sum += v[r];
      const float mu = sum / 32.f;
      float m2 = 0.f;
#pragma unroll
      for (int r = 0; r < 32; ++r) { const float d = v[r] - mu; m2 += d * d; }
      stats[(long)(base >> 5) * 64 + c] = make_float2(sum, m2);
    } else if (cnt > 0) {
      float sum = 0.f;
      for (int r = 0; r < cnt; ++r) sum += T[(32 * grp + r) * LDT + c];
      const float mu = sum / (float)cnt;
      float m2 = 0.f;
      for (int r = 0; r < cnt; ++r) { const float d = T[(32 * grp + r) * LDT + c] - mu; m2 += d * d; }
      stats[(long)(base >> 5) * 64 + c] = make_float2(sum, m2);
    }
  }
// ... 683 lines not shown
```

### yolat_vectorgraphicsrecognition_amd/csrc/forward_eval.hip

```cpp
#include "common.hpp"

namespace {
struct Plan {
  int* row_ptr; int* perm; int* src; int* dst; float* attr; int* work; int* seg_ptr; int* node_seg;
  float* H1; float* H2; float* UV; float* UV2; float* f_tmp[YOLAT_MAX_LAYERS]; float* s_tmp[YOLAT_MAX_LAYERS];
  float* feats; float* fsup; float* Z; float* c1; float* c2;
  float* gx_work;
  uint16_t* Zs;
  size_t bytes;
};

Plan carve(const yolat_model_eval* m, long N, long E, long P, void* ws) {
  Carver c{reinterpret_cast<char*>(ws), 0};
  Plan p;
  const long C = m->C, F = m->F, D = C * m->n_blocks_out, Ee = E > 0 ? E : 1;
  p.row_ptr = c.take<int>(N + 1); p.perm = c.take<int>(Ee); p.src = c.take<int>(Ee); p.dst = c.take<int>(Ee);
  p.attr = c.take<float>(Ee * 4); p.work = c.take<int>(yolat_graph_work_elems(N, E));
  p.seg_ptr = c.take<int>(P + 1); p.node_seg = c.take<int>(N);
  p.H1 = c.take<float>(Ee * C); p.H2 = c.take<float>(Ee * C); p.UV = c.take<float>(N * 2 * C);
  p.UV2 = (m->n_blocks >= 2 && yl_edge_tile_groups(N, E) == 1) ? c.take<float>(N * 2 * C) : nullptr;
  const int lo = m->n_blocks - m->n_blocks_out;
  for (int l = 0; l < m->n_blocks; ++l) {
    p.f_tmp[l] = (l < lo) ? c.take<float>(N * C) : nullptr;
    p.s_tmp[l] = (l < lo) ? c.take<float>(N * C) : nullptr;
  }
  p.feats = c.take<float>(N * D); p.fsup = c.take<float>(N * D);
  p.Z = c.take<float>(P * 2 * (F + D)); p.c1 = c.take<float>(P * m->H1); p.c2 = c.take<float>(P * m->H2);
  const size_t gxw = (m->Wc1_gx && (2 * (F + D)) % 16 == 0) ? yolat_gemm_x6_work_elems(P, m->H1, 2 * (F + D)) : 0;
  p.gx_work = gxw ? c.take<float>((long)gxw) : nullptr;
  p.Zs = (P <= YOLAT_CLS_X6_MAX_ROWS && m->Wc_x6[0] && (2 * (F + D)) % 16 == 0)
             ? c.take<uint16_t>((long)yolat_split_bf16x3_packed_elems(P, 2 * (F + D))) : nullptr;
  p.bytes = c.off + 256;
  return p;
}
}

static int prep_node_uv(const int64_t* edge, int64_t stride_e, int64_t stride_c, const float* e_attr,
                        const int64_t* bbox_idx, int64_t E, int64_t N, int64_t P, const Plan& p, int32_t* status,
                        const float* x, int64_t ldx, int64_t Cin, const float* Wuv, const float* uv_bias, const float* Wr,
                        const float* br, const float* Wn, const float* bn, const float* sn, const float* tn, int64_t C,
                        float* f_out, int64_t ld_fo, float* s_out, int64_t ld_so, bool primed, yolat_stream_t stream) {
  NodeUv a;
  const int rc = yl_build_node_uv(&a, x, ldx, x, ldx, N, Cin, Wuv, uv_bias, Wr, br, Wn, bn, sn, tn, C, p.UV, 2 * C, f_out,
                                  ld_fo, s_out, ld_so);
  if (rc != 0) return rc;
  return yl_graph_prepare_impl(edge, stride_e, stride_c, e_attr, bbox_idx, E, N, P, p.row_ptr, p.perm, p.src, p.dst,
                               p.attr, p.seg_ptr, p.node_seg, p.work, status, &a, primed, stream);
}

#include <stdlib.h>
#include <string>
#include <vector>
namespace {
struct StageRec { std::string name; double flops, bytes; std::vector<std::pair<hipEvent_t, hipEvent_t>> ev; };
std::vector<StageRec> g_stages;
std::vector<hipEvent_t> g_pool;
bool g_profile = false;
hipEvent_t new_event() {
  if (!g_pool.empty()) { hipEvent_t e = g_pool.back(); g_pool.pop_back(); return e; }
  hipEvent_t e; (void)hipEventCreate(&e); return e;
}
StageRec& stage_rec(const char* name, double flops, double bytes) {
  for (auto& s : g_stages) if (s.name == name) { s.flops += flops; s.bytes += bytes; return s; }
  g_stages.push_back(StageRec{name, flops, bytes, {}});
  return g_stages.back();
}
}

#define YL_STAGE(name, flops, bytes, call)                         \
  do {                                                                      \
    if (g_profile) {                                                        \
      StageRec& sr__ = stage_rec(name, (double)(flops), (double)(bytes));   \
      hipEvent_t a__ = new_event(), b__ = new_event();                      \
      (void)hipEventRecord(a__, (hipStream_t)stream);                       \
      int rc__ = (call);                                                    \
      (void)hipEventRecord(b__, (hipStream_t)stream);                       \
      sr__.ev.push_back({a__, b__});                                        \
      if (rc__ != 0) return rc__;                                           \
    } else {                                                                \
      YL_TRY(call);                                                         \
    }                                                                       \
  } while (0)

namespace { int g_open_stage = -1; }
bool yl_profile_on() { return g_profile; }
void yl_stage_begin(const char* name, double flops, double bytes, yolat_stream_t stream) {
  stage_rec(name, flops, bytes);
  for (size_t i = 0; i < g_stages.size(); ++i) if (g_stages[i].name == name) g_open_stage = (int)i;
  hipEvent_t a = new_event(), b = new_event();
  (void)hipEventRecord(a, (hipStream_t)stream);
  g_stages[g_open_stage].ev.push_back({a, b});
}
void yl_stage_end(yolat_stream_t stream) {
  if (g_open_stage >= 0) (void)hipEventRecord(g_stages[g_open_stage].ev.back().second, (hipStream_t)stream);
  g_open_stage = -1;
}

extern "C" int yolat_profile_enable(int on) { g_profile = on != 0; return 0; }
extern "C" int yolat_profile_enabled(void) { return g_profile ? 1 : 0; }
extern "C" int yolat_profile_reset(void) {
  for (auto& s : g_stages) for (auto& e : s.ev) { g_pool.push_back(e.first); g_pool.push_back(e.second); }
  g_stages.clear();
  return 0;
}
extern "C" int yolat_profile_count(void) { return (int)g_stages.size(); }
extern "C" int yolat_profile_get(int index, char* name, int cap, float* total_ms, int* calls, double* flops,
                                 double* bytes) {
  if (index < 0 || index >= (int)g_stages.size() || !name || cap <= 0) return YOLAT_E_INVALID;
  StageRec& s = g_stages[index];
  snprintf(name, cap, "%s", s.name.c_str());
  float tot = 0.f;
  for (auto& e : s.ev) { float ms = 0.f; if (hipEventElapsedTime(&ms, e.first, e.second) == hipSuccess) tot += ms; }
  if (total_ms) *total_ms = tot;
  if (calls) *calls = (int)s.ev.size();
  const double n = s.ev.empty() ? 1.0 : (double)s.ev.size();
  if (flops) *flops = s.flops / n;
  if (bytes) *bytes = s.bytes / n;
  return 0;
}

static int cls1_x6(const float* Z, long ZW, long P, uint16_t* Zs, const uint16_t* Wp, const float* shift, long H1,
                   float* c1, yolat_stream_t stream) {
  YL_TRY(yolat_split_bf16x3_packed(Z, ZW, P, ZW, nullptr, Zs, stream));
  return yolat_linear_x6_pre(Zs, P, ZW, Wp, shift, 1, H1, c1, H1, stream);
}

extern "C" size_t yolat_forward_eval_workspace_bytes(const yolat_model_eval* m, int64_t N, int64_t E,
                                                     int64_t P) {
  if (!m || N <= 0 || E < 0 || P <= 0) return 0;
  return carve(m, N, E, P, nullptr).bytes;
}

static int forward_eval_impl(const yolat_model_eval* m, const float* x, int64_t ldx, const int64_t* edge,
                             int64_t stride_e, int64_t stride_c, const float* e_attr, const int64_t* bbox_idx,
                             int64_t N, int64_t E, int64_t P, float* logits, int64_t ld_logits, void* workspace,
                             size_t workspace_bytes, int32_t* status, bool primed, yolat_stream_t stream,
                             const yolat_graph_csr* g = nullptr);

extern "C" int yolat_forward_eval_csr(const yolat_model_eval* m, const float* x, int64_t ldx, const yolat_graph_csr* g,
                                      int64_t N, int64_t E, int64_t P, float* logits, int64_t ld_logits, void* workspace,
                                      size_t workspace_bytes, yolat_stream_t stream) {
  YL_TRY(yl_adopt_graph<Plan>(g, E, nullptr));
  int32_t unused_status = 0;
  return forward_eval_impl(m, x, ldx, nullptr, 0, 0, nullptr, reinterpret_cast<const int64_t*>(g->node_seg), N, E, P, logits,
                           ld_logits, workspace, workspace_bytes, &unused_status, false, stream, g);
}

extern "C" int yolat_forward_eval(const yolat_model_eval* m, const float* x, int64_t ldx,
                                  const int64_t* edge, int64_t stride_e, int64_t stride_c,
                                  const float* e_attr, const int64_t* bbox_idx, int64_t N, int64_t E,
                                  int64_t P, float* logits, int64_t ld_logits, void* workspace,
                                  size_t workspace_bytes, int32_t* status, yolat_stream_t stream) {
  return forward_eval_impl(m, x, ldx, edge, stride_e, stride_c, e_attr, bbox_idx, N, E, P, logits, ld_logits, workspace,
                           workspace_bytes, status, false, stream);
}

extern "C" int yolat_forward_eval_primed(const yolat_model_eval* m, const float* x, int64_t ldx,
                                         const int64_t* edge, int64_t stride_e, int64_t stride_c,
                                         const float* e_attr, const int64_t* bbox_idx, int64_t N, int64_t E,
                                         int64_t P, float* logits, int64_t ld_logits, void* workspace,
                                         size_t workspace_bytes, int32_t* status, yolat_stream_t stream) {
  return forward_eval_impl(m, x, ldx, edge, stride_e, stride_c, e_attr, bbox_idx, N, E, P, logits, ld_logits, workspace,
                           workspace_bytes, status, true, stream);
}

static int forward_eval_impl(const yolat_model_eval* m, const float* x, int64_t ldx, const int64_t* edge,
                             int64_t stride_e, int64_t stride_c, const float* e_attr, const int64_t* bbox_idx,
                             int64_t N, int64_t E, int64_t P, float* logits, int64_t ld_logits, void* workspace,
                             size_t workspace_bytes, int32_t* status, bool primed, yolat_stream_t stream,
                             const yolat_graph_csr* g) {
  if (!m || !x || !bbox_idx || !logits || !workspace || !status || N <= 0 || E < 0 || P <= 0)
    return YOLAT_E_INVALID;
  if (m->n_blocks < 1 || m->n_blocks > YOLAT_MAX_LAYERS || m->n_blocks_out < 1 ||
      m->n_blocks_out > m->n_blocks)
    return YOLAT_E_INVALID;
  Plan p = carve(m, N, E, P, workspace);
  if (p.bytes > workspace_bytes) return YOLAT_E_INVALID;
  if (g != nullptr) YL_TRY(yl_adopt_graph(g, E, &p));
  const long C = m->C, F = m->F, D = C * m->n_blocks_out, ZW = 2 * (F + D);
  const int lo = m->n_blocks - m->n_blocks_out;

  char nm[128];
  const yolat_conv_eval& cv0 = m->conv[0];
  const bool node0_ok = C == 64 && cv0.Wuv != nullptr && cv0.Wc4 != nullptr;
  const bool node0_in_prep = node0_ok && g == nullptr;
  const bool fold0 = cv0.Wuvf && cv0.uvb && cv0.Wc4f && cv0.t2f;
  static const bool chain_on = []() { const char* v = getenv("YOLAT_NODE_CHAIN"); return !(v && v[0] == '0'); }();
  bool chain_mode = chain_on && node0_ok && fold0 && E > 0 && m->n_blocks >= 2 && p.UV2 != nullptr &&
                    yl_edge_tile_groups(N, E) == 1;
  for (int l = 1; l < m->n_blocks && chain_mode; ++l) {
    const yolat_conv_eval& c = m->conv[l];
    chain_mode = c.Cin == 64 && c.Wuv && c.Wc4 && c.Wuvf && c.uvb && c.Wc4f && c.t2f && c.Wnx && c.tnx && c.Wn &&
                 c.sn && c.tn && yl_aligned16(c.Wn);
  }
  bool next_done = false;
  float* uv_next = nullptr;
  if (node0_in_prep) {
    const int slot0 = 0 - lo;
    float* f0 = slot0 >= 0 ? p.feats + slot0 * C : p.f_tmp[0];
    float* s0 = slot0 >= 0 ? p.fsup + slot0 * C : p.s_tmp[0];
    const long ld0 = slot0 >= 0 ? D : C;
    YL_STAGE("graph_prep[csr+attr+segments] + node_uv[layer 0]", 8.0 * N * cv0.Cin * C,
             16.0 * E + 12.0 * E + 32.0 * E + 12.0 * N + 4.0 * (2.0 * N * cv0.Cin + 4.0 * N * C),
             prep_node_uv(edge, stride_e, stride_c, e_attr, bbox_idx, E, N, P, p, status, x, ldx, cv0.Cin,
                          fold0 ? cv0.Wuvf : cv0.Wuv, fold0 ? cv0.uvb : nullptr, cv0.Wr, cv0.br, cv0.Wn, cv0.bn, cv0.sn,
                          cv0.tn, C, f0, ld0, s0, ld0, primed, stream));
  } else if (g == nullptr) {
  YL_STAGE("graph_prep[csr+attr+segments]", 0, 16.0 * E + 12.0 * E + 32.0 * E + 12.0 * N,
           yl_graph_prepare_impl(edge, stride_e, stride_c, e_attr, bbox_idx, E, N, P, p.row_ptr, p.perm, p.src,
                                 p.dst, p.attr, p.seg_ptr, p.node_seg, p.work, status, nullptr, primed, stream));
  }

  static const bool riders_on = []() { const char* v = getenv("YOLAT_POOL_RIDERS"); return !(v && v[0] == '0'); }();
  const bool fusion_x6 = m->Wf_hi && m->Wf_mid && m->Wf_lo && m->tf_fold && m->Wfs_hi && m->Wfs_mid && m->Wfs_lo &&
                         m->tfs_fold && (D == 64 || D == 128) && F % 64 == 0 && (long)P * ZW < (1LL << 32);
  const bool small_pool = riders_on && (long)P * (F + 2 * D) <= (1L << 20);
  PoolRider ride_a{}, ride_b{};
  ride_a.feats = ride_b.feats = p.feats; ride_a.fsup = ride_b.fsup = p.fsup; ride_a.ld = ride_b.ld = D;
  ride_a.D = ride_b.D = (int)D; ride_a.F = ride_b.F = (int)F; ride_a.P = ride_b.P = (int)P;
  ride_a.seg_ptr = ride_b.seg_ptr = p.seg_ptr; ride_a.Z = ride_b.Z = p.Z; ride_a.ldz = ride_b.ldz = ZW;
  ride_a.parts = YL_POOL_ZERO | YL_POOL_MEAN; ride_a.blocks = small_pool && fusion_x6 ? 256 : 0;
  ride_b.parts = YL_POOL_MAX; ride_b.blocks = small_pool && fusion_x6 ? 64 : 0;
  int pool_done = 0;

  const float* f_in = x; long ld_f = ldx;
  const float* s_in = x; long ld_s = ldx;
  for (int l = 0; l < m->n_blocks; ++l) {
    const yolat_conv_eval& cv = m->conv[l];
    const int slot = l - lo;
    float* f_out = slot >= 0 ? p.feats + slot * C : p.f_tmp[l];
    float* s_out = slot >= 0 ? p.fsup + slot * C : p.s_tmp[l];
    const long ld_out = slot >= 0 ? D : C;
    const double K1 = 2.0 * cv.Cin + 4;
    if (C == 64) {
      if (cv.Wuv != nullptr && cv.Wc4 != nullptr) {
        const bool fold = cv.Wuvf && cv.uvb && cv.Wc4f && cv.t2f;
        float* uv_l = next_done ? uv_next : p.UV;
        if (!(l == 0 && node0_in_prep) && !next_done) {
          uv_l = p.UV;
          snprintf(nm, sizeof nm, "node_uv[UV | lin_r | mlp_node, N x %ld -> %ld+%ld+%ld]", (long)cv.Cin, 2 * C, C, C);
          const bool node_x6 = fold && cv.Cin == 64 && N >= YOLAT_NODE_X6_MIN_ROWS && cv.Wfr_x6[0] && cv.Wfr_x6[1] &&
                               cv.Wfr_x6[2] && cv.tfr && cv.Wn_x6[0] && cv.Wn_x6[1] && cv.Wn_x6[2] && cv.tn_fold &&
                               ld_f % 4 == 0 && ld_s % 4 == 0;
          YL_STAGE(nm, 8.0 * N * cv.Cin * C, 4.0 * (2.0 * N * cv.Cin + 4.0 * N * C),
                   node_x6 ? yolat_node_uv_eval_x6(f_in, ld_f, s_in, ld_s, N, cv.Wfr_x6[0], cv.Wfr_x6[1], cv.Wfr_x6[2],
                                                   cv.tfr, cv.Wn_x6[0], cv.Wn_x6[1], cv.Wn_x6[2], cv.tn_fold, p.UV, 2 * C,
                                                   f_out, ld_out, s_out, ld_out, stream)
                           : yolat_node_uv_eval(f_in, ld_f, s_in, ld_s, N, cv.Cin, fold ? cv.Wuvf : cv.Wuv,
                                                fold ? cv.uvb : nullptr, cv.Wr, cv.br, cv.Wn, cv.bn, cv.sn, cv.tn, C, p.UV,
                                                2 * C, f_out, ld_out, s_out, ld_out, stream));
        }
        if (E > 0) {
          const PoolRider* rd = (l == m->n_blocks - 1 && ride_a.blocks > 0) ? &ride_a : nullptr;
          int rode = 0, did_next = 0;
          EdgeNext nx{};
          if (chain_mode && l + 1 < m->n_blocks) {
            const int sn = l + 1 - lo;
            nx.Wp = m->conv[l + 1].Wnx; nx.bias = m->conv[l + 1].tnx;
            nx.UV = (uv_l == p.UV) ? p.UV2 : p.UV; nx.ld_uv = 2 * C;
            nx.root = sn >= 0 ? p.feats + sn * C : p.f_tmp[l + 1]; nx.ld_root = sn >= 0 ? D : C;
            const yolat_conv_eval& cn = m->conv[l + 1];
            nx.s_in = s_out; nx.ld_si = ld_out;
            nx.Wn = cn.Wn; nx.bn = cn.bn; nx.sn = cn.sn; nx.tn = cn.tn;
            nx.s_out = sn >= 0 ? p.fsup + sn * C : p.s_tmp[l + 1]; nx.ld_so = sn >= 0 ? D : C;
            nx.s_tiles = yl_cdiv(N, 64);
          }
          const bool with_next = nx.Wp != nullptr;
          if (with_next)
            snprintf(nm, sizeof nm, "edge_uv_mlp2_mean+node_uv_next[E x (U+V+attr) -> %ld -> %ld -> mean; N x %ld -> %ld+%ld+%ld]",
                     C, C, C, 2 * C, C, C);
          else
            snprintf(nm, sizeof nm, "edge_uv_mlp2_mean[E x (U+V+attr) -> %ld -> %ld -> mean]", C, C);
          YL_STAGE(nm, 2.0 * E * (4.0 * C + C * C) + (with_next ? 8.0 * N * C * C : 0.0),
                   E * ((2.0 * cv.Cin + 4.0) * 4.0 + 8.0) + 4.0 * N * C + (with_next ? 4.0 * (N * C + 4.0 * N * C) : 0.0),
                   fold ? yl_edge_uv_mlp2_mean_eval_impl(uv_l, 2 * C, p.src, p.dst, p.attr, p.row_ptr, N, E, cv.Wc4f,
                                                         nullptr, nullptr, nullptr, cv.W2, nullptr, cv.s2, cv.t2f, C,
                                                         f_out, ld_out, YOLAT_EDGE_AUTO, rd, &rode,
                                                         nx.Wp ? &nx : nullptr, &did_next, stream)
                        : yl_edge_uv_mlp2_mean_eval_impl(uv_l, 2 * C, p.src, p.dst, p.attr, p.row_ptr, N, E, cv.Wc4,
                                                         cv.b1, cv.s1, cv.t1, cv.W2, cv.b2, cv.s2, cv.t2, C, f_out,
                                                         ld_out, YOLAT_EDGE_AUTO, rd, &rode, nullptr, nullptr, stream));
          if (rode) pool_done |= ride_a.parts;
          next_done = did_next != 0;
          uv_next = nx.UV;
        }
      } else {
      if (E > 0) {
        snprintf(nm, sizeof nm, "edge_mlp2[E x %ld -> %ld -> %ld, gathered]", (long)K1, C, C);
        YL_STAGE(nm, 2.0 * E * (K1 * C + C * C), E * (K1 * 4.0 + 8.0) + 4.0 * E * C,
                 yolat_edge_mlp2_eval(f_in, ld_f, N, cv.Cin, p.src, p.dst, p.attr, E, cv.W1, cv.b1, cv.s1, cv.t1,
                                      cv.W2, cv.b2, cv.s2, cv.t2, C, p.H2, C, stream));
      }
      snprintf(nm, sizeof nm, "node_pair[lin_r | mlp_node, N x %ld -> %ld]", (long)cv.Cin, C);
      YL_STAGE(nm, 4.0 * N * cv.Cin * C, 8.0 * (N * cv.Cin + N * C),
               yolat_node_side_eval(f_in, ld_f, s_in, ld_s, N, cv.Cin, cv.Wr, cv.br, cv.Wn, cv.bn, cv.sn, cv.tn,
                                    nullptr, C, p.row_ptr, 0, C, f_out, ld_out, s_out, ld_out, stream));
      if (E > 0) {
        YL_STAGE("csr_mean[E x C -> N x C]", 1.0 * E * C, 4.0 * (E * C + 2.0 * N * C) + 4.0 * N,
                 yolat_csr_mean_fwd(p.H2, C, C, nullptr, nullptr, 0, p.row_ptr, N, f_out, ld_out, 1, stream));
      }
      }
    } else {
    snprintf(nm, sizeof nm, "lin_r[N x %ld -> %ld]", (long)cv.Cin, C);
    YL_STAGE(nm, 2.0 * N * cv.Cin * C, 4.0 * (N * cv.Cin + N * C + C * cv.Cin),
             yolat_linear_fwd(f_in, ld_f, N, cv.Cin, nullptr, nullptr, 0, cv.Wr, cv.Cin, cv.br, C, nullptr,
                              nullptr, 0, f_out, ld_out, 0, nullptr, stream));
    if (E > 0) {
      snprintf(nm, sizeof nm, "edge_lin1[E x %ld -> %ld, gathered]", (long)K1, C);
      YL_STAGE(nm, 2.0 * E * K1 * C, E * (K1 * 4.0 + 8.0) + 4.0 * E * C,
               yolat_edge_lin1_fwd(f_in, ld_f, N, cv.Cin, p.src, p.dst, p.attr, E, cv.W1, 2 * cv.Cin + 4,
                                   cv.b1, C, cv.s1, cv.t1, 1, p.H1, C, nullptr, stream));
      snprintf(nm, sizeof nm, "edge_lin2[E x %ld -> %ld]", C, C);
      YL_STAGE(nm, 2.0 * E * C * C, 8.0 * E * C,
               yolat_linear_fwd(p.H1, C, E, C, nullptr, nullptr, 0, cv.W2, C, cv.b2, C, cv.s2, cv.t2, 1, p.H2,
                                C, 0, nullptr, stream));
      YL_STAGE("csr_mean[E x C -> N x C]", 1.0 * E * C, 4.0 * (E * C + 2.0 * N * C) + 4.0 * N,
               yolat_csr_mean_fwd(p.H2, C, C, nullptr, nullptr, 0, p.row_ptr, N, f_out, ld_out, 1, stream));
    }
    snprintf(nm, sizeof nm, "mlp_node[N x %ld -> %ld]", (long)cv.Cin, C);
    YL_STAGE(nm, 2.0 * N * cv.Cin * C, 4.0 * (N * cv.Cin + N * C + C * cv.Cin),
             yolat_linear_fwd(s_in, ld_s, N, cv.Cin, nullptr, nullptr, 0, cv.Wn, cv.Cin, cv.bn, C, cv.sn, cv.tn, 1,
                              s_out, ld_out, 0, nullptr, stream));
    }
    f_in = f_out; ld_f = ld_out; s_in = s_out; ld_s = ld_out;
  }

  float* sup = p.Z + 2 * F + D;
  const bool ride_max = ride_b.blocks > 0 && (pool_done & YL_POOL_ZERO);
  const int pool_left = (YL_POOL_ZERO | YL_POOL_MAX | YL_POOL_MEAN) & ~pool_done & ~(ride_max ? YL_POOL_MAX : 0);
  if (pool_left) {
    YL_STAGE("pool_prepare[max(feats), mean(fsup), zero]", 2.0 * N * D, 8.0 * N * D + 4.0 * P * (F + 2 * D),
             yl_pool_prepare_parts(p.feats, p.fsup, D, D, F, p.seg_ptr, P, p.Z, ZW, pool_left, stream));
  }
  snprintf(nm, sizeof nm, "fusion_gemm+segmax[N x %ld -> %ld -> P] | super[P x %ld -> %ld]", D, F, D, F);
  YL_STAGE(nm, 2.0 * (N + P) * D * F, 4.0 * (N * D + 2.0 * D * F + 2.0 * P * F + N + P * D),
           fusion_x6 ? yl_fusion_pair_eval_x6_impl(p.feats, D, N, D, m->Wf_hi, m->Wf_mid, m->Wf_lo, m->tf_fold, F,
                                                   p.node_seg, p.Z, ZW, sup, ZW, P, m->Wfs_hi, m->Wfs_mid, m->Wfs_lo,
                                                   m->tfs_fold, p.Z + F + D, ZW, ride_max ? &ride_b : nullptr, stream)
                     : yolat_fusion_pair_eval(p.feats, D, N, D, m->Wf, m->bf, m->sf, m->tf, F, p.node_seg, p.Z, ZW, sup,
                                              ZW, P, m->Wfs, m->bfs, m->sfs, m->tfs, p.Z + F + D, ZW, stream));
  bool cls_x6 = p.Zs != nullptr && m->H1 % 16 == 0 && m->H2 % 16 == 0;
  for (int i = 0; i < 3; ++i) cls_x6 = cls_x6 && m->Wc_x6[i] != nullptr && m->tc_fold[i] != nullptr;
  const bool cls1_gx = m->Wc1_gx && m->tc1_gx && ZW % 16 == 0 && P >= YOLAT_CLS1_X6_MIN_ROWS;
  static const bool sk_x6_on = []() { const char* v = getenv("YOLAT_CLS1_SK_X6"); return !(v && v[0] == '0'); }();
  const bool cls1_sk = sk_x6_on && !cls1_gx && !cls_x6 && !yl_strict_fp32() && ZW >= 1024 && ZW % 128 == 0 &&
                       (long)yl_cdiv(P, 64) * yl_cdiv(m->H1, 64) < 160 && yl_aligned16(p.Z) && yl_aligned16(m->Wc1);
  snprintf(nm, sizeof nm, "cls1[P x %ld -> %ld]", ZW, (long)m->H1);
  YL_STAGE(nm, 2.0 * P * ZW * m->H1, 4.0 * (P * ZW + ZW * m->H1 + P * m->H1),
           cls1_gx ? yolat_gemm_x6(p.Z, ZW, P, ZW, m->Wc1_gx, m->tc1_gx, 1, m->H1, p.c1, m->H1, p.gx_work, stream)
           : cls_x6 ? cls1_x6(p.Z, ZW, P, p.Zs, m->Wc_x6[0], m->tc_fold[0], m->H1, p.c1, stream)
           : cls1_sk ? yolat_linear_sk_x6(p.Z, ZW, P, ZW, m->Wc1, ZW, m->bc1, m->H1, m->sc1, m->tc1, 1, p.c1, m->H1, stream)
                  : yolat_linear_fwd(p.Z, ZW, P, ZW, nullptr, nullptr, 0, m->Wc1, ZW, m->bc1, m->H1, m->sc1, m->tc1, 1,
                                     p.c1, m->H1, 0, nullptr, stream));
  snprintf(nm, sizeof nm, "cls2[P x %ld -> %ld]", (long)m->H1, (long)m->H2);
  YL_STAGE(nm, 2.0 * P * m->H1 * m->H2, 4.0 * (P * m->H1 + m->H1 * m->H2 + P * m->H2),
           cls_x6 ? yolat_linear_x6(p.c1, m->H1, P, m->H1, m->Wc_x6[1], m->tc_fold[1], 1, m->H2, p.c2, m->H2, stream)
                  : yolat_linear_fwd(p.c1, m->H1, P, m->H1, nullptr, nullptr, 0, m->Wc2, m->H1, m->bc2, m->H2, m->sc2,
                                     m->tc2, 1, p.c2, m->H2, 0, nullptr, stream));
  snprintf(nm, sizeof nm, "cls3[P x %ld -> %d]", (long)m->H2, (int)m->n_classes);
  YL_STAGE(nm, 2.0 * P * m->H2 * m->n_classes, 4.0 * (P * m->H2 + m->H2 * m->n_classes + P * m->n_classes),
           cls_x6 ? yolat_linear_x6(p.c2, m->H2, P, m->H2, m->Wc_x6[2], m->tc_fold[2], 0, m->n_classes, logits,
                                    ld_logits, stream)
                  : yolat_linear_fwd(p.c2, m->H2, P, m->H2, nullptr, nullptr, 0, m->Wc3, m->H2, m->bc3, m->n_classes,
                                     nullptr, nullptr, 0, logits, ld_logits, 0, nullptr, stream));
// ... 3 lines not shown
```

### yolat_vectorgraphicsrecognition_amd/csrc/graph.hip

```cpp
#include "common.hpp"

__global__ void k_edge_count(const int64_t* edge, long se, long sc, int E, int N, int* src32,
                             int* dst32, int* cnt, int* status) {
  const int e = blockIdx.x * blockDim.x + threadIdx.x;
  if (e >= E) return;
  int64_t s = edge[(long)e * se];
  int64_t d = edge[(long)e * se + sc];
  if (s < 0 || s >= N || d < 0 || d >= N) {
    atomicOr(status, YOLAT_STATUS_EDGE_RANGE);
    s = s < 0 ? 0 : (s >= N ? N - 1 : s);
    d = d < 0 ? 0 : (d >= N ? N - 1 : d);
  }
  src32[e] = (int)s; dst32[e] = (int)d;
  atomicAdd(&cnt[d], 1);
}

__global__ void k_count32(const int* key, int n, int* cnt) {
  const int i = blockIdx.x * blockDim.x + threadIdx.x;
  if (i >= n) return;
  const int k = key[i];
  if (k >= 0) atomicAdd(&cnt[k], 1);
}

__global__ void __launch_bounds__(1024) k_scan_excl(int* cnt, int N, int* ptr) {
// ... 502 lines not shown
  const bool last = (int)blockIdx.x == g.nprep - 1;
  if (tid < PS_RMAX) { rowcnt[tid] = 0; cur[tid] = 0; }
  if (tid == 0) list_n = 0;
  __syncthreads();
  int below = 0;
  ps_walk<0>(g, r0, r1, rowcnt, nullptr, nullptr, &list_n, list, below, 0, nullptr);
#pragma unroll
  for (int off = 32; off > 0; off >>= 1) below += __shfl_down(below, off);
  if (lane == 0) wbelow[w] = below;
  __syncthreads();
  const int rt = tid < PS_RMAX ? rowcnt[tid] : 0;
  int incl = rt;
#pragma unroll
  for (int off = 1; off < 64; off <<= 1) {
    const int nb = __shfl_up(incl, off);
    if (lane >= off) incl += nb;
  }
  if (tid < PS_RMAX && lane == 63) wtot[w] = incl;
  int base = 0;
#pragma unroll
  for (int v = 0; v < PS_NW; ++v) base += wbelow[v];
  const int n_list = list_n;
  __syncthreads();
  if (tid < PS_RMAX) {
    int off = 0;
#pragma unroll
    for (int v = 0; v < PS_RMAX / 64; ++v) off += (v < w) ? wtot[v] : 0;
    rowstart[tid] = off + incl - rt;
    if (r0 + tid < r1) g.row_ptr[r0 + tid] = base + off + incl - rt;
    if (last && tid == PS_RMAX - 1) g.row_ptr[g.N] = base + off + incl;
  }
  if (n_list <= PS_CAP) {
    static_assert(PS_CAP == 4 * PS_T, "four list entries per thread, spelled out");
    __syncthreads();
    for (int i = tid; i < n_list; i += PS_T) {
      const unsigned en = list[i];
      const int dl = (int)(en >> 20);
      grp[rowstart[dl] + atomicAdd(&cur[dl], 1)] = en;
    }
    __syncthreads();
    if (n_list > 0) {
      const int lastv = n_list - 1;
      auto emit_k = [&](int i, unsigned en, int64_t sv, float a0, float a1, float a2, float a3) {
        if (i >= n_list) return;
        const int dl = (int)(en >> 20), b = rowstart[dl], n = rowcnt[dl];
        int r = 0;
        for (int u = 0; u < n; ++u) r += (grp[b + u] < en) ? 1 : 0;
        if (sv < 0 || sv >= g.N) { atomicOr(g.status, YOLAT_STATUS_EDGE_RANGE); sv = sv < 0 ? 0 : g.N - 1; }
        const int pos = base + b + r;
        g.perm[pos] = (int)(en & 0xFFFFFu);
        g.src_csr[pos] = (int)sv;
        g.dst_csr[pos] = r0 + dl;
        g.attr_csr[pos] = make_float4(a0, a1, a2, a3);
      };
#define PS_G(k)                                                                        \
      const unsigned en##k = list[yl_min(tid + (k) * PS_T, lastv)];                    \
      const int64_t sx##k = g.edge[(long)(en##k & 0xFFFFFu) * g.se];                   \
      const float4 ax##k = g.attr[en##k & 0xFFFFFu];
      PS_G(0) PS_G(1) PS_G(2) PS_G(3)
#undef PS_G
      emit_k(tid, en0, sx0, ax0.x, ax0.y, ax0.z, ax0.w);
      emit_k(tid + PS_T, en1, sx1, ax1.x, ax1.y, ax1.z, ax1.w);
      emit_k(tid + 2 * PS_T, en2, sx2, ax2.x, ax2.y, ax2.z, ax2.w);
      emit_k(tid + 3 * PS_T, en3, sx3, ax3.x, ax3.y, ax3.z, ax3.w);
    }
  } else {
    __syncthreads();
    for (int i = tid; i < PS_NW * PS_RMAX; i += PS_T) { (&cnt[0][0])[i] = 0; (&msk[0][0])[i] = 0ull; }
    __syncthreads();
    int unused = 0;
    ps_walk<1>(g, r0, r1, nullptr, cnt[w], msk[w], nullptr, nullptr, unused, 0, nullptr);
    __syncthreads();
    if (tid < PS_RMAX) {
      int run = 0;
#pragma unroll
      for (int v = 0; v < PS_NW; ++v) { const int t = cnt[v][tid]; cnt[v][tid] = run; run += t; }
    }
    __syncthreads();
    ps_walk<2>(g, r0, r1, nullptr, cnt[w], msk[w], nullptr, nullptr, unused, base, rowstart);
  }
}

#define PS_PLAN_ROWS 100
#define PS_PLAN_EDGES (PS_CAP / 2)
#define PS_PLAN_GRID 250
static int prep_small_rows(int64_t N, int64_t E, int64_t other_blocks) {
  static const bool on = []() { const char* e = getenv("YOLAT_PREP_SMALL"); return !(e && e[0] == '0'); }();
  static const int forced = []() { const char* e = getenv("YOLAT_PREP_R"); const int r = e ? atoi(e) : 0;
                                   return (r >= 1 && r <= PS_RMAX) ? r : 0; }();
  if (!on || N <= 0 || E < 0 || E > 98304) return 0;
  if (forced) return forced;
  int64_t r_edges = E > 0 ? (int64_t)PS_PLAN_EDGES * N / E : PS_RMAX;
  if (r_edges < 1) r_edges = 1;
  int64_t R = PS_PLAN_ROWS;
  if (R > r_edges) R = r_edges;
  if (R > N) R = N;
  if ((N + R - 1) / R + other_blocks > PS_PLAN_GRID) {
    const int64_t room = PS_PLAN_GRID - other_blocks;
    if (room < 1) return 0;
    R = (N + room - 1) / room;
    if (R > PS_RMAX || R > r_edges) return 0;
  }
  return (int)R;
}

extern "C" int yolat_graph_prepare_plan(int64_t N, int64_t E, int64_t other_wgs, int32_t* rows, int32_t* csr_wgs) {
  const int R = (other_wgs < 0) ? 0 : prep_small_rows(N, E, other_wgs);
  if (rows) *rows = R;
  if (csr_wgs) *csr_wgs = R > 0 ? (int32_t)((N + R - 1) / R) : 0;
  return R > 0 ? 1 : 0;
}

extern "C" size_t yolat_graph_work_elems(int64_t N, int64_t E) {
  return (size_t)(2 * (((N + 1) + 63) / 64 * 64) + 4 * E + (N + 1) / PREP_BLK + 16);
}

int yl_graph_prepare_impl(const int64_t* edge, int64_t stride_e, int64_t stride_c, const float* e_attr,
                              const int64_t* bbox_idx, int64_t E, int64_t N, int64_t P, int32_t* row_ptr,
                              int32_t* perm, int32_t* src_csr, int32_t* dst_csr, float* attr_csr, int32_t* seg_ptr,
                              int32_t* node_seg, int32_t* work, int32_t* status, const NodeUv* extra, bool primed,
                              yolat_stream_t stream) {
  if (N <= 0 || E < 0 || N >= (1LL << 31) - 8192 || E >= (1LL << 31) - 256) return YOLAT_E_INVALID;
  if (!row_ptr || !work || !status) return YOLAT_E_INVALID;
  if (E > 0 && (!edge || !e_attr || !perm || !src_csr || !dst_csr || !attr_csr)) return YOLAT_E_INVALID;
  if (bbox_idx && (P <= 0 || !seg_ptr || !node_seg)) return YOLAT_E_INVALID;
  if (E > 0 && !yl_aligned16(e_attr)) return YOLAT_E_UNSUPPORTED;
  hipStream_t st = (hipStream_t)stream;
  const int n1 = (int)N + 1;
  const int nblk = yl_cdiv(n1, PREP_BLK);
  const int n1p = (n1 + 63) / 64 * 64;
  int* cnt = work;
  int* local = cnt + n1p;
  int* btot = local + n1p;
  int* src32 = btot + nblk + 1;
  int* dst32 = src32 + E;
  int* rank = dst32 + E;
  int* items = rank + E;
  const int node_blocks = extra ? yl_cdiv(extra->N, 8 * PS_NW * PS_NODE_ITERS) : 0;
  const int seg_blocks = bbox_idx ? yl_cdiv(N + 1, PS_T) : 0;
  const int Rs = (extra == nullptr || yl_node3_smallk_shape_ok(*extra)) ? prep_small_rows(N, E, node_blocks + seg_blocks) : 0;
  if (Rs > 0) {
    PrepSmall g;
    g.edge = edge; g.se = (long)stride_e; g.sc = (long)stride_c; g.attr = reinterpret_cast<const float4*>(e_attr);
    g.bbox = bbox_idx; g.P = (long)P; g.E = (int)E; g.N = (int)N; g.R = Rs; g.nprep = yl_cdiv(N, Rs);
    g.nseg = seg_blocks;
    g.row_ptr = row_ptr; g.perm = perm; g.src_csr = src_csr; g.dst_csr = dst_csr;
    g.attr_csr = reinterpret_cast<float4*>(attr_csr); g.seg_ptr = seg_ptr; g.node_seg = node_seg; g.status = status;
    NodeUv none{};
    hipLaunchKernelGGL(k_prep_small, dim3(g.nprep + g.nseg + node_blocks), dim3(PS_T), 0, st, g, extra ? *extra : none,
                       extra ? 1 : 0);
    YL_LAUNCH_CHECK();
    return 0;
  }
  if (!primed) {
    hipLaunchKernelGGL(k_zero_i32, dim3(yl_cdiv(n1p, 1024)), dim3(256), 0, st, cnt, n1p);
    YL_LAUNCH_CHECK();
  }
  const long nthreads = (E > N + 1) ? E : N + 1;
  hipLaunchKernelGGL(k_prep_count_win, dim3(yl_cdiv(nthreads, PCW_E)), dim3(PCW_T), 0, st, edge, (long)stride_e,
                     (long)stride_c, (int)E, (int)N, src32, dst32, rank, cnt, bbox_idx, (long)P, seg_ptr,
                     node_seg, status);
  YL_LAUNCH_CHECK();
  hipLaunchKernelGGL(k_prep_scan, dim3(nblk), dim3(1024), 0, st, cnt, n1, local, btot);
  YL_LAUNCH_CHECK();
  if (E > 0) {
    hipLaunchKernelGGL(k_prep_fill, dim3(yl_cdiv(E, 256)), dim3(256), 0, st, dst32, rank, (int)E, local, btot,
                       items);
    YL_LAUNCH_CHECK();
  }
  const int rows_blocks = yl_cdiv(E > n1 ? E : n1, 256);
  if (extra != nullptr && yl_node3_smallk_ok(*extra)) {
    hipLaunchKernelGGL(k_prep_rows, dim3(rows_blocks), dim3(256), 0, st, local, btot, (int)N, (int)E, items, src32, dst32,
                       reinterpret_cast<const float4*>(e_attr), row_ptr, perm, src_csr, dst_csr,
                       reinterpret_cast<float4*>(attr_csr));
    YL_LAUNCH_CHECK();
    return yl_node3_smallk(*extra, st);
  }
  if (extra != nullptr) {
    const unsigned total = (unsigned)rows_blocks + 4u * (unsigned)yl_cdiv(extra->N, 64);
    if (extra->Cin <= 16)
      hipLaunchKernelGGL(k_prep_rows_node3<16>, dim3(total), dim3(256), 0, st, local, btot, (int)N, (int)E, items, src32, dst32,
                         reinterpret_cast<const float4*>(e_attr), row_ptr, perm, src_csr, dst_csr,
                         reinterpret_cast<float4*>(attr_csr), rows_blocks, *extra);
    else
      hipLaunchKernelGGL(k_prep_rows_node3<32>, dim3(total), dim3(256), 0, st, local, btot, (int)N, (int)E, items, src32, dst32,
                         reinterpret_cast<const float4*>(e_attr), row_ptr, perm, src_csr, dst_csr,
                         reinterpret_cast<float4*>(attr_csr), rows_blocks, *extra);
  } else {
    hipLaunchKernelGGL(k_prep_rows, dim3(rows_blocks), dim3(256), 0, st, local, btot, (int)N, (int)E, items, src32, dst32,
                       reinterpret_cast<const float4*>(e_attr), row_ptr, perm, src_csr, dst_csr,
                       reinterpret_cast<float4*>(attr_csr));
  }
  YL_LAUNCH_CHECK();
  return 0;
}

extern "C" int yolat_graph_prepare(const int64_t* edge, int64_t stride_e, int64_t stride_c,
                                   const float* e_attr, const int64_t* bbox_idx, int64_t E, int64_t N,
                                   int64_t P, int32_t* row_ptr, int32_t* perm, int32_t* src_csr,
                                   int32_t* dst_csr, float* attr_csr, int32_t* seg_ptr, int32_t* node_seg,
                                   int32_t* work, int32_t* status, yolat_stream_t stream) {
  return yl_graph_prepare_impl(edge, stride_e, stride_c, e_attr, bbox_idx, E, N, P, row_ptr, perm, src_csr, dst_csr,
                            attr_csr, seg_ptr, node_seg, work, status, nullptr, false, stream);
}

extern "C" int yolat_graph_prepare_node_uv(const int64_t* edge, int64_t stride_e, int64_t stride_c,
                                           const float* e_attr, const int64_t* bbox_idx, int64_t E, int64_t N,
                                           int64_t P, int32_t* row_ptr, int32_t* perm, int32_t* src_csr,
                                           int32_t* dst_csr, float* attr_csr, int32_t* seg_ptr, int32_t* node_seg,
                                           int32_t* work, int32_t* status, const float* x, int64_t ldx, int64_t Cin,
                                           const float* Wuv, const float* uv_bias, const float* Wr, const float* br,
                                           const float* Wn,
                                           const float* bn, const float* sn, const float* tn, int64_t C, float* UV,
                                           int64_t ld_uv, float* f_out, int64_t ld_fo, float* s_out, int64_t ld_so,
                                           yolat_stream_t stream) {
  NodeUv a;
  const int rc = yl_build_node_uv(&a, x, ldx, x, ldx, N, Cin, Wuv, uv_bias, Wr, br, Wn, bn, sn, tn, C, UV, ld_uv, f_out,
                                  ld_fo, s_out, ld_so);
  if (rc != 0) return rc;
  return yl_graph_prepare_impl(edge, stride_e, stride_c, e_attr, bbox_idx, E, N, P, row_ptr, perm, src_csr, dst_csr,
                            attr_csr, seg_ptr, node_seg, work, status, &a, false, stream);
}

// ... 22 lines not shown
```

### yolat_vectorgraphicsrecognition_amd/ops.py

```python
import ctypes
import os

import torch

from ._lib import lib, check

STATS_ROWS = 32
STATUS_EDGE_RANGE, STATUS_SEG_UNSORTED, STATUS_SEG_RANGE, STATUS_NOT_LOCAL = 1, 2, 4, 8

_WEIGHT_EPOCH = [0]


def weight_epoch():
    return _WEIGHT_EPOCH[0]


def bump_weight_epoch():
    _WEIGHT_EPOCH[0] += 1


_RAW_STREAM = getattr(torch._C, "_cuda_getCurrentRawStream", None)
_GET_DEVICE = getattr(torch._C, "_cuda_getDevice", None)
_STREAM_OBJ = {}

# ... 553 lines not shown
    N, Cin = x.shape
    C = W1.shape[0]
    g.ensure_csc()
    if wuv is None:
        wuv, _ = split_w1(W1, Cin)
    dwc4_done = None
    if partial is not None:
        dUV, dwc4_done = partial
        check(lib.yolat_edge_uv_sums_v(dH1.data_ptr(), _ld(dH1), int(_is_h(dH1)), g.col_ptr.data_ptr(), g.slots.data_ptr(),
                                       N, C, dUV.data_ptr(), 2 * C, _stream()), "yolat_edge_uv_sums_v")
    else:
        dUV = torch.empty(N, 2 * C, dtype=torch.float32, device=x.device)
        if _is_h(dH1):
            check(lib.yolat_edge_uv_sums_h(_h(dH1), _ld(dH1), g.row_ptr.data_ptr(), g.col_ptr.data_ptr(),
                                           g.slots.data_ptr(), N, C, dUV.data_ptr(), 2 * C, _stream()),
                  "yolat_edge_uv_sums_h")
        else:
            check(lib.yolat_edge_uv_sums(_f(dH1), _ld(dH1), g.row_ptr.data_ptr(), g.col_ptr.data_ptr(),
                                         g.slots.data_ptr(), N, C, dUV.data_ptr(), 2 * C, _stream()), "yolat_edge_uv_sums")
    def weight_grads():
        dwuv = torch.empty(2 * C, Cin, dtype=torch.float32, device=x.device)
        linear_bwd_w(dUV, x, dwuv)
        if dwc4_done is not None:
            dwc4 = dwc4_done
        else:
            dwc4 = torch.empty(C, 4, dtype=torch.float32, device=x.device)
            attr_dw(dH1, g, dwc4, db1)
        check(lib.yolat_conv_merge_dw1(dwuv.data_ptr(), dwc4.data_ptr(), Cin, C, _f(dW1), _ld(dW1), 0, _stream()),
              "yolat_conv_merge_dw1")
    if side is not None:
        side(weight_grads, (dUV, x, dH1, g.attr, dwc4_done))
    else:
        weight_grads()
    if dx is not None:
        linear_fwd_wt(dUV, wuv, dx, accumulate=dx_accumulate)
    return dW1


def edge_lin1_fwd_factorised(x, g, W1, b1, H1, stats=None, keep=None):
    N, Cin = x.shape
    C = W1.shape[0]
    wuv, wc4 = split_w1(W1, Cin)
    if keep is not None:
        keep["wuv"] = wuv
    uv = torch.empty(N, 2 * C, dtype=torch.float32, device=x.device)
    linear_fwd(x, wuv, None, uv)
    if _is_h(H1):
        check(lib.yolat_edge_uv_lin1_fwd_h(uv.data_ptr(), 2 * C, g.src.data_ptr(), g.dst.data_ptr(), g.attr.data_ptr(),
                                           g.E, wc4.data_ptr(), _f(b1, "b1", True), C, _h(H1, "H1"), _ld(H1),
                                           _f(stats, "stats", True), _stream()), "yolat_edge_uv_lin1_fwd_h")
        return H1
    check(lib.yolat_edge_uv_lin1_fwd(uv.data_ptr(), 2 * C, g.src.data_ptr(), g.dst.data_ptr(), g.attr.data_ptr(), g.E,
                                     wc4.data_ptr(), _f(b1, "b1", True), C, _f(H1), _ld(H1),
                                     _f(stats, "stats", True), _stream()), "yolat_edge_uv_lin1_fwd")
    return H1


def fold_factorised_layer(wuv, wc4, b1, s1, t1, b2, s2, t2):
    zeros = torch.zeros_like(s1)
    b1 = zeros if b1 is None else b1.detach()
    b2 = zeros if b2 is None else b2.detach()
    wuvf = (wuv * torch.cat([s1, s1]).unsqueeze(1)).contiguous()
    uvb = torch.cat([s1 * b1 + t1, zeros]).contiguous()
    wc4f = (wc4 * s1.unsqueeze(1)).contiguous()
    t2f = (s2 * b2 + t2).contiguous()
    return wuvf, uvb, wc4f, t2f


EDGE_AUTO, EDGE_TILES, EDGE_WS_F32, EDGE_WS_X6 = 0, 1, 2, 3


def edge_uv_mlp2_mean_eval(UV, g, wc4, b1, pro1, W2, b2, pro2, f_out, variant=EDGE_AUTO):
    s1, t1 = pro1 if pro1 is not None else (None, None)
    s2, t2 = pro2 if pro2 is not None else (None, None)
    check(lib.yolat_edge_uv_mlp2_mean_eval_variant(_f(UV, "UV"), _ld(UV), g.src.data_ptr(), g.dst.data_ptr(),
                                                   g.attr.data_ptr(), g.row_ptr.data_ptr(), g.N, g.E, _f(wc4),
                                                   _f(b1, "b1", True), _f(s1, "s1", True), _f(t1, "t1", True), _f(W2),
                                                   _f(b2, "b2", True), _f(s2, "s2", True), _f(t2, "t2", True),
                                                   W2.shape[0], _f(f_out), _ld(f_out), int(variant), _stream()),
          "yolat_edge_uv_mlp2_mean_eval_variant")
    return f_out


def edge_mlp2_eval(x, g, W1, b1, pro1, W2, b2, pro2, H2):
    N, Cin = x.shape
    C = W1.shape[0]
    if not (W1.is_contiguous() and W2.is_contiguous()):
        raise ValueError("W1 / W2 must be contiguous")
    check(lib.yolat_edge_mlp2_eval(_f(x, "x"), _ld(x), N, Cin, g.src.data_ptr(), g.dst.data_ptr(), g.attr.data_ptr(),
                                   g.E, _f(W1), _f(b1), _f(pro1[0]), _f(pro1[1]), _f(W2), _f(b2), _f(pro2[0]),
                                   _f(pro2[1]), C, _f(H2), _ld(H2), _stream()), "yolat_edge_mlp2_eval")
    return H2


def edge_lin1_bwd_w(dH1, x, g, dW1, db1=None, accumulate=False):
    E, C = dH1.shape[0], dW1.shape[0]
    N, Cin = x.shape
    work = torch.empty(int(lib.yolat_linear_bwd_w_work_elems(g.E, C, 2 * Cin + 4)), dtype=torch.float32,
                       device=x.device)
    check(lib.yolat_edge_lin1_bwd_w(_f(dH1), _ld(dH1), g.E, C, _f(x), _ld(x), N, Cin, g.src.data_ptr(),
                                    g.dst.data_ptr(), g.attr.data_ptr(), _f(dW1), _ld(dW1),
                                    _f(db1, "db1", True), int(accumulate), work.data_ptr(), _stream()),
          "yolat_edge_lin1_bwd_w")
    return dW1


def edge_lin1_bwd_x(dH1, W1, Cin, dG):
    C = W1.shape[0]
    check(lib.yolat_edge_lin1_bwd_x(_f(dH1), _ld(dH1), dH1.shape[0], C, _f(W1), _ld(W1), Cin, _f(dG),
                                    _ld(dG), _stream()), "yolat_edge_lin1_bwd_x")
    return dG


def edge_scatter_bwd(dG, Cin, g, dX, accumulate=False):
    g.ensure_csc()
    check(lib.yolat_edge_scatter_bwd(_f(dG), _ld(dG), Cin, g.row_ptr.data_ptr(), g.col_ptr.data_ptr(),
                                     g.slots.data_ptr(), g.N, _f(dX), _ld(dX), int(accumulate),
                                     _stream()), "yolat_edge_scatter_bwd")
    return dX


def csr_mean_fwd(H, g, out, h_pro=None, h_relu=False, accumulate=False):
    C = out.shape[1]
    hs, hb = (h_pro if h_pro is not None else (None, None))
    if _is_h(H):
        check(lib.yolat_csr_mean_fwd_h(_h(H, "H"), _ld(H), C, _f(hs, "h_scale", True), _f(hb, "h_shift", True),
                                       int(h_relu), g.row_ptr.data_ptr(), g.N, _f(out), _ld(out), int(accumulate),
                                       _stream()), "yolat_csr_mean_fwd_h")
        return out
    check(lib.yolat_csr_mean_fwd(_f(H, "H", g.E == 0), _ld(H) if H is not None else C, C,
                                 _f(hs, "h_scale", True), _f(hb, "h_shift", True), int(h_relu),
                                 g.row_ptr.data_ptr(), g.N, _f(out), _ld(out), int(accumulate),
                                 _stream()), "yolat_csr_mean_fwd")
    return out


def csr_mean_bwd(dOut, g, dM):
    C = dOut.shape[1]
    if _is_h(dM):
        check(lib.yolat_csr_mean_bwd_h(_f(dOut), _ld(dOut), C, g.row_ptr.data_ptr(), g.dst.data_ptr(), g.E, _h(dM, "dM"),
                                       _ld(dM), _stream()), "yolat_csr_mean_bwd_h")
        return dM
    check(lib.yolat_csr_mean_bwd(_f(dOut), _ld(dOut), C, g.row_ptr.data_ptr(), g.dst.data_ptr(), g.E,
                                 _f(dM), _ld(dM), _stream()), "yolat_csr_mean_bwd")
    return dM



def segment_mean_fwd(X, g, Y, x_pro=None, x_relu=False):
    D = X.shape[1]
    xs, xb = (x_pro if x_pro is not None else (None, None))
    check(lib.yolat_segment_mean_fwd(_f(X), _ld(X), D, _f(xs, "x_scale", True), _f(xb, "x_shift", True),
                                     int(x_relu), g.seg_ptr.data_ptr(), g.P, _f(Y), _ld(Y), _stream()),
          "yolat_segment_mean_fwd")
    return Y


def segment_max_fwd(X, g, Y, arg=None, x_pro=None, x_relu=False):
    D = X.shape[1]
    xs, xb = (x_pro if x_pro is not None else (None, None))
    check(lib.yolat_segment_max_fwd(_f(X), _ld(X), D, _f(xs, "x_scale", True), _f(xb, "x_shift", True),
                                    int(x_relu), g.seg_ptr.data_ptr(), g.P, g.N, _f(Y), _ld(Y),
                                    _i(arg, torch.int32, "arg"), _stream()), "yolat_segment_max_fwd")
    return Y


# ... 294 lines not shown
```

Before: 16740.

## Add throughput regime with multi-tile edge kernel and larger prep row blocks

Adds a per-process regime detector that watches how many streams called forward eval within a recent time window. When several streams run at once it switches to a throughput regime. In that regime the edge MLP+mean kernel processes several node tiles per workgroup, and graph prep uses larger row blocks, so fewer, fatter workgroups are launched and W2 staging is amortised across tiles. This trades single-call latency for lower per-workgroup overhead under concurrency, and relies on a timing heuristic that may misclassify.

New measurement: 17390 (median of 6 runs). 1.04x the previous value.

```diff
diff --git a/include/yolat_hip.h b/include/yolat_hip.h
--- a/include/yolat_hip.h
+++ b/include/yolat_hip.h
@@ -57,6 +57,8 @@
                         yolat_stream_t stream);
 
 int yolat_graph_prepare_plan(int64_t N, int64_t E, int64_t other_wgs, int32_t* rows, int32_t* csr_wgs);
+int yolat_graph_prepare_plan_regime(int64_t N, int64_t E, int64_t other_wgs, int regime, int32_t* rows,
+                                    int32_t* csr_wgs);
 
 int yolat_gather_rows(const float* src, int64_t ld_src, const int32_t* idx, int64_t rows,
                       int64_t width, float* dst, int64_t ld_dst, yolat_stream_t stream);
@@ -176,6 +178,12 @@
                                          const float* t1, const float* W2, const float* b2, const float* s2,
                                          const float* t2, int64_t C, float* f_out, int64_t ld_fo, int variant,
                                          yolat_stream_t stream);
+#define YOLAT_EDGE_MT_MAX 16
+int yolat_edge_uv_mlp2_mean_eval_mt(const float* UV, int64_t ld_uv, const int32_t* src_csr, const int32_t* dst_csr,
+                                    const float* attr_csr, const int32_t* row_ptr, int64_t N, int64_t E,
+                                    const float* Wc4, const float* b1, const float* s1, const float* t1,
+                                    const float* W2, const float* b2, const float* s2, const float* t2, int64_t C,
+                                    float* f_out, int64_t ld_fo, int tiles_per_wg, yolat_stream_t stream);
 int yolat_edge_uv_mlp2_eval(const float* UV, int64_t ld_uv, const int32_t* src_csr, const int32_t* dst_csr,
                             const float* attr_csr, int64_t E, const float* Wc4, const float* b1, const float* s1,
                             const float* t1, const float* W2, const float* b2, const float* s2, const float* t2,
@@ -311,6 +319,11 @@
                               const int64_t* bbox_idx, int64_t N, int64_t E, int64_t P, float* logits,
                               int64_t ld_logits, void* workspace, size_t workspace_bytes, int32_t* status,
                               yolat_stream_t stream);
+
+int yolat_eval_regime_observe(uint64_t stream_key, uint64_t now_ns);
+int yolat_eval_regime_set(int mode);
+int yolat_eval_regime_get(void);
+int yolat_eval_regime_counts(int64_t out[2]);
 
 typedef struct { const void* ptr; int64_t bytes; } yolat_span;
 int yolat_collate_pack(void* dst, const int64_t* field_off, const yolat_span* spans, int64_t n_fields, int64_t n_items);
diff --git a/yolat_vectorgraphicsrecognition_amd/_lib.py b/yolat_vectorgraphicsrecognition_amd/_lib.py
--- a/yolat_vectorgraphicsrecognition_amd/_lib.py
+++ b/yolat_vectorgraphicsrecognition_amd/_lib.py
@@ -148,6 +148,8 @@
                                               c_p, c_p, c_i64, c_p, c_i64, c_p]),
     "yolat_edge_uv_mlp2_mean_eval_variant": (c_int, [c_p, c_i64, c_p, c_p, c_p, c_p, c_i64, c_i64, c_p, c_p, c_p, c_p,
                                                       c_p, c_p, c_p, c_p, c_i64, c_p, c_i64, c_int, c_p]),
+    "yolat_edge_uv_mlp2_mean_eval_mt": (c_int, [c_p, c_i64, c_p, c_p, c_p, c_p, c_i64, c_i64, c_p, c_p, c_p, c_p,
+                                                 c_p, c_p, c_p, c_p, c_i64, c_p, c_i64, c_int, c_p]),
     "yolat_edge_uv_sums": (c_int, [c_p, c_i64, c_p, c_p, c_p, c_i64, c_i64, c_p, c_i64, c_p]),
     "yolat_conv_merge_dw1": (c_int, [c_p, c_p, c_i64, c_i64, c_p, c_i64, c_int, c_p]),
     "yolat_fusion_pair_eval": (c_int, [c_p, c_i64, c_i64, c_i64, c_p, c_p, c_p, c_p, c_i64, c_p, c_p, c_i64, c_p, c_i64,
@@ -161,6 +163,11 @@
     "yolat_graph_prepare": (c_int, [c_p, c_i64, c_i64, c_p, c_p, c_i64, c_i64, c_i64, c_p, c_p, c_p, c_p, c_p,
                                     c_p, c_p, c_p, c_p, c_p]),
     "yolat_graph_prepare_plan": (c_int, [c_i64, c_i64, c_i64, c_p, c_p]),
+    "yolat_graph_prepare_plan_regime": (c_int, [c_i64, c_i64, c_i64, c_int, c_p, c_p]),
+    "yolat_eval_regime_observe": (c_int, [ctypes.c_uint64, ctypes.c_uint64]),
+    "yolat_eval_regime_set": (c_int, [c_int]),
+    "yolat_eval_regime_get": (c_int, []),
+    "yolat_eval_regime_counts": (c_int, [c_p]),
     "yolat_gather_rows": (c_int, [c_p, c_i64, c_p, c_i64, c_i64, c_p, c_i64, c_p]),
     "yolat_bn_stats_elems": (c_sz, [c_i64, c_i64]),
     "yolat_linear_fwd": (c_int, [c_p, c_i64, c_i64, c_i64, c_p, c_p, c_int,
diff --git a/yolat_vectorgraphicsrecognition_amd/csrc/common.hpp b/yolat_vectorgraphicsrecognition_amd/csrc/common.hpp
--- a/yolat_vectorgraphicsrecognition_amd/csrc/common.hpp
+++ b/yolat_vectorgraphicsrecognition_amd/csrc/common.hpp
@@ -800,7 +800,7 @@
                                    const float* b1, const float* s1, const float* t1, const float* W2, const float* b2,
                                    const float* s2, const float* t2, int64_t C, float* f_out, int64_t ld_fo, int variant,
                                    const PoolRider* rider, int* rode, const EdgeNext* next, int* did_next,
-                                   yolat_stream_t stream);
+                                   yolat_stream_t stream, int tiles_per_wg = 1);
 int yl_fusion_pair_eval_x6_impl(const float* A, int64_t lda, int64_t N, int64_t D, const uint16_t* Wh, const uint16_t* Wm,
                                 const uint16_t* Wl, const float* tfold, int64_t F, const int32_t* node_seg, float* pool,
                                 int64_t ldpool, const float* S, int64_t lds, int64_t P, const uint16_t* Wsh,
@@ -821,10 +821,13 @@
                   int32_t* seg_ptr, int32_t* node_seg, int32_t* eptr, int32_t* status, int32_t* info, bool vouched,
                   hipStream_t st);
 
+#define YL_REGIME_LATENCY 0
+#define YL_REGIME_THROUGHPUT 1
 int yl_graph_prepare_impl(const int64_t* edge, int64_t stride_e, int64_t stride_c, const float* e_attr,
                           const int64_t* bbox_idx, int64_t E, int64_t N, int64_t P, int32_t* row_ptr, int32_t* perm,
                           int32_t* src_csr, int32_t* dst_csr, float* attr_csr, int32_t* seg_ptr, int32_t* node_seg,
-                          int32_t* work, int32_t* status, const NodeUv* extra, bool primed, yolat_stream_t stream);
+                          int32_t* work, int32_t* status, const NodeUv* extra, bool primed, yolat_stream_t stream,
+                          int regime = YL_REGIME_LATENCY);
 template <int BK>
 __device__ __forceinline__ void node_uv_tile(const NodeUv& a, int x, int y) {
   if (y < 2) gemm_nt_tile<64, 64, BK, DenseOp, DenseOp, false>(a.af, a.wuv, a.euv, a.N, 2 * a.C, a.Cin, x, y);
diff --git a/yolat_vectorgraphicsrecognition_amd/csrc/edge.hip b/yolat_vectorgraphicsrecognition_amd/csrc/edge.hip
--- a/yolat_vectorgraphicsrecognition_amd/csrc/edge.hip
+++ b/yolat_vectorgraphicsrecognition_amd/csrc/edge.hip
@@ -467,6 +467,267 @@
 #ifdef YOLAT_EDGE_STAMPS
   if (threadIdx.x == 0 && blockIdx.x < 4096) edge_stamps_d[nx.Wp != nullptr ? 0 : 1][blockIdx.x * 16 + 11] = (long long)((e1g - e0g + 63) / 64);
 #endif
+}
+
+constexpr int EDGE_LDH = 65;
+struct EdgeL1 { float4 wc[4]; float4 bb, sc, sh; };
+__device__ __forceinline__ void edge_l1_consts(EdgeL1& k, const float* __restrict__ Wc4, const float* __restrict__ b1,
+                                               const float* __restrict__ s1, const float* __restrict__ t1, int q) {
+#pragma unroll
+  for (int j = 0; j < 4; ++j) k.wc[j] = *reinterpret_cast<const float4*>(Wc4 + (4 * q + j) * 4);
+  k.bb = b1 ? *reinterpret_cast<const float4*>(b1 + 4 * q) : make_float4(0.f, 0.f, 0.f, 0.f);
+  k.sc = make_float4(1.f, 1.f, 1.f, 1.f); k.sh = make_float4(0.f, 0.f, 0.f, 0.f);
+  if (s1) { k.sc = *reinterpret_cast<const float4*>(s1 + 4 * q); k.sh = *reinterpret_cast<const float4*>(t1 + 4 * q); }
+}
+__device__ __forceinline__ void edge_w2_load(const DenseOp& W2, int tid, float (&rw2)[4][4]) {
+#pragma unroll
+  for (int t = 0; t < 4; ++t) {
+    const int i = tid + t * 256;
+    W2.template load4<false>(i >> 4, 4 * (i & 15), rw2[t]);
+  }
+}
+__device__ __forceinline__ void edge_w2_store(float* W2s, int tid, const float (&rw2)[4][4]) {
+#pragma unroll
+  for (int t = 0; t < 4; ++t) {
+    const int i = tid + t * 256;
+    float* d = W2s + (i >> 4) * EDGE_LDH + 4 * (i & 15);
+    d[0] = rw2[t][0]; d[1] = rw2[t][1]; d[2] = rw2[t][2]; d[3] = rw2[t][3];
+  }
+}
+__device__ __forceinline__ void edge_gather_layer1(const float* __restrict__ UV, long ld_uv, const float* __restrict__ attr,
+                                                   int c0, int E, int rb, int q, const int (&di)[4], const int (&si)[4],
+                                                   const EdgeL1& k, float* Hs) {
+  float4 u[4], v[4], a[4];
+#pragma unroll
+  for (int t = 0; t < 4; ++t) {
+    const int e = yl_min(c0 + rb + 16 * t, E - 1);
+    u[t] = *reinterpret_cast<const float4*>(UV + (long)di[t] * ld_uv + 4 * q);
+    v[t] = *reinterpret_cast<const float4*>(UV + (long)si[t] * ld_uv + 64 + 4 * q);
+    a[t] = *reinterpret_cast<const float4*>(attr + (long)e * 4);
+  }
+#pragma unroll
+  for (int t = 0; t < 4; ++t) {
+    auto one = [&](float uu, float vv, const float4& w, float b, float s, float h) {
+      float z = uu + vv;
+      z = fmaf(a[t].x, w.x, z); z = fmaf(a[t].y, w.y, z); z = fmaf(a[t].z, w.z, z); z = fmaf(a[t].w, w.w, z);
+      return fmaxf(fmaf(z + b, s, h), 0.f);
+    };
+    float* hrow = Hs + (rb + 16 * t) * EDGE_LDH + 4 * q;
+    hrow[0] = one(u[t].x, v[t].x, k.wc[0], k.bb.x, k.sc.x, k.sh.x);
+    hrow[1] = one(u[t].y, v[t].y, k.wc[1], k.bb.y, k.sc.y, k.sh.y);
+    hrow[2] = one(u[t].z, v[t].z, k.wc[2], k.bb.z, k.sc.z, k.sh.z);
+    hrow[3] = one(u[t].w, v[t].w, k.wc[3], k.bb.w, k.sc.w, k.sh.w);
+  }
+}
+__device__ __forceinline__ f32x16 edge_mfma_tile(const float* Hs, const float* W2s, int wm, int wn, int l31, int lhi) {
+  f32x16 acc;
+#pragma unroll
+  for (int r = 0; r < 16; ++r) acc[r] = 0.f;
+#pragma unroll 8
+  for (int kk = 0; kk < 64; kk += 2) {
+    const float av = Hs[(wm * 32 + l31) * EDGE_LDH + kk + lhi];
+    const float bv = W2s[(wn * 32 + l31) * EDGE_LDH + kk + lhi];
+    acc = __builtin_amdgcn_mfma_f32_32x32x2f32(av, bv, acc, 0, 0, 0);
+  }
+  return acc;
+}
+__device__ __forceinline__ void edge_store_messages(const f32x16& acc2, float* Hs, int wm, int lhi, int col, float bias2,
+                                                    float sc2, float sh2) {
+#pragma unroll
+  for (int r = 0; r < 16; ++r) {
+    const int row = wm * 32 + (r & 3) + 8 * (r >> 2) + 4 * lhi;
+    Hs[row * EDGE_LDH + col] = fmaxf(fmaf(acc2[r] + bias2, sc2, sh2), 0.f);
+  }
+}
+template <int NG>
+__device__ __forceinline__ void edge_aggregate(const float* Hs, int c0, int rb, int q, int nn, const int (&my_b)[NG],
+                                               const int (&my_e)[NG], float4 (&sum)[NG]) {
+#pragma unroll
+  for (int j = 0; j < NG; ++j) {
+    if (rb + 16 * j < nn) {
+      const int lo = my_b[j] > c0 ? my_b[j] : c0;
+      const int hi = my_e[j] < c0 + 64 ? my_e[j] : c0 + 64;
+      for (int e = lo; e < hi; ++e) {
+        const float* m = Hs + (e - c0) * EDGE_LDH + 4 * q;
+        sum[j].x += m[0]; sum[j].y += m[1]; sum[j].z += m[2]; sum[j].w += m[3];
+      }
+    }
+  }
+}
+template <int NG>
+__device__ __forceinline__ void edge_mean_out(float* f_out, long ld_fo, int n0, int rb, int q, int nn, const int (&my_b)[NG],
+                                              const int (&my_e)[NG], const float4 (&sum)[NG], float4 (&fo)[NG]) {
+#pragma unroll
+  for (int j = 0; j < NG; ++j) {
+    const int deg = my_e[j] - my_b[j];
+    if (rb + 16 * j < nn && deg > 0) {
+      const float inv = 1.f / (float)deg;
+      float4* o = reinterpret_cast<float4*>(f_out + (long)(n0 + rb + 16 * j) * ld_fo + 4 * q);
+      float4 d = fo[j];
+      d.x = yl_mul_rn(sum[j].x, inv) + d.x; d.y = yl_mul_rn(sum[j].y, inv) + d.y;
+      d.z = yl_mul_rn(sum[j].z, inv) + d.z; d.w = yl_mul_rn(sum[j].w, inv) + d.w;
+      *o = d;
+      fo[j] = d;
+    }
+  }
+}
+__device__ __forceinline__ void edge_s_tile(const EdgeNext& nx, int N, int r0, float* Hs, float* W2s, int tid, int wm, int wn,
+                                            int l31, int lhi) {
+#pragma unroll
+  for (int t = 0; t < 4; ++t) {
+    const int i = tid + t * 256, row = i >> 4, c4 = 4 * (i & 15);
+    const float4 av = *reinterpret_cast<const float4*>(nx.s_in + (long)yl_min(r0 + row, N - 1) * nx.ld_si + c4);
+    const float4 wv = *reinterpret_cast<const float4*>(nx.Wn + row * 64 + c4);
+    float* da = Hs + row * EDGE_LDH + c4;
+    float* dw = W2s + row * EDGE_LDH + c4;
+    da[0] = av.x; da[1] = av.y; da[2] = av.z; da[3] = av.w;
+    dw[0] = wv.x; dw[1] = wv.y; dw[2] = wv.z; dw[3] = wv.w;
+  }
+  const int colS = wn * 32 + l31;
+  const float bS = nx.bn ? nx.bn[colS] : 0.f, scS = nx.sn[colS], shS = nx.tn[colS];
+  __syncthreads();
+  const f32x16 accS = edge_mfma_tile(Hs, W2s, wm, wn, l31, lhi);
+#pragma unroll
+  for (int r = 0; r < 16; ++r) {
+    const int row = r0 + wm * 32 + (r & 3) + 8 * (r >> 2) + 4 * lhi;
+    if (row < N) nx.s_out[(long)row * nx.ld_so + colS] = fmaxf(fmaf(accS[r] + bS, scS, shS), 0.f);
+  }
+}
+__device__ __forceinline__ void edge_next_node_side(const EdgeNext& nx, int n0, int nn, int rb, int q, int wave, int lane,
+                                                    const float4& fo0, float* Hs) {
+  float bfa[16], bfb[16];
+#pragma unroll
+  for (int ks = 0; ks < 16; ++ks) bfa[ks] = nx.Wp[(wave * 16 + ks) * 64 + lane];
+  float* frow = Hs + rb * EDGE_LDH + 4 * q;
+  const float4 fz = (rb < nn) ? fo0 : make_float4(0.f, 0.f, 0.f, 0.f);
+  frow[0] = fz.x; frow[1] = fz.y; frow[2] = fz.z; frow[3] = fz.w;
+  __syncthreads();
+  const int fr = lane & 15, fk = lane >> 4;
+#pragma unroll
+  for (int t = 0; t < 3; ++t) {
+    const int ct = wave + 4 * t;
+    if (t < 2) {
+#pragma unroll
+      for (int ks = 0; ks < 16; ++ks) bfb[ks] = nx.Wp[((ct + 4) * 16 + ks) * 64 + lane];
+    }
+    const int col = ct * 16 + fr;
+    const float bias = nx.bias[col];
+    f32x4 acc = {0.f, 0.f, 0.f, 0.f};
+#pragma unroll
+    for (int ks = 0; ks < 16; ++ks)
+      acc = __builtin_amdgcn_mfma_f32_16x16x4f32(Hs[fr * EDGE_LDH + 4 * ks + fk], bfa[ks], acc, 0, 0, 0);
+#pragma unroll
+    for (int r = 0; r < 4; ++r) {
+      const int row = 4 * fk + r;
+      if (row < nn) {
+        const float v = acc[r] + bias;
+        if (col < 128) nx.UV[(long)(n0 + row) * nx.ld_uv + col] = v;
+        else nx.root[(long)(n0 + row) * nx.ld_root + (col - 128)] = v;
+      }
+    }
+#pragma unroll
+    for (int ks = 0; ks < 16; ++ks) bfa[ks] = bfb[ks];
+  }
+}
+
+template <bool NEXT>
+__global__ void __launch_bounds__(256, 4) k_edge_mt_uv_mlp2_mean(const float* __restrict__ UV, long ld_uv,
+                                                                 const int* __restrict__ src, const int* __restrict__ dst,
+                                                                 const float* __restrict__ attr,
+                                                                 const int* __restrict__ row_ptr, int N, int npt,
+                                                                 const float* __restrict__ Wc4, const float* __restrict__ b1,
+                                                                 const float* __restrict__ s1, const float* __restrict__ t1,
+                                                                 DenseOp W2, const float* __restrict__ b2,
+                                                                 const float* __restrict__ s2, const float* __restrict__ t2,
+                                                                 float* f_out, long ld_fo, int E, int tiles, int T, int wgs,
+                                                                 PoolRider rider, EdgeNext nx) {
+  if ((int)blockIdx.x >= wgs + nx.s_tiles) {
+    yl_pool_rider(rider, blockIdx.x - wgs - nx.s_tiles, rider.blocks, threadIdx.x, 256);
+    return;
+  }
+  constexpr int LDH = EDGE_LDH;
+  __shared__ float Hs[64 * LDH];
+  __shared__ float W2s[64 * LDH];
+  __shared__ int ahead[2][64 + 64 + 17];
+  const int tid = threadIdx.x, wave = tid >> 6, lane = tid & 63;
+  const int wm = wave >> 1, wn = wave & 1, l31 = lane & 31, lhi = lane >> 5;
+  if (NEXT && (int)blockIdx.x >= wgs) {
+    edge_s_tile(nx, N, (blockIdx.x - wgs) * 64, Hs, W2s, tid, wm, wn, l31, lhi);
+    return;
+  }
+  const int q = tid & 15, rb = tid >> 4;
+  const int col = wn * 32 + l31;
+  const int tA = blockIdx.x * T, tB = yl_min(tA + T, tiles);
+  auto start_load = [&](int nA, int eA) -> int {
+    if (tid < 64) return dst[yl_min(eA + tid, E - 1)];
+    if (tid < 128) return src[yl_min(eA + tid - 64, E - 1)];
+    if (tid < 145) return row_ptr[yl_min(nA + tid - 128, nA + yl_min(npt, N - nA))];
+    return 0;
+  };
+  {
+    const int n0 = tA * npt;
+    const int e0g = row_ptr[n0];
+    const int st = start_load(n0, e0g);
+    float rw2[4][4];
+    edge_w2_load(W2, tid, rw2);
+    if (tid < 145) ahead[0][tid] = st;
+    edge_w2_store(W2s, tid, rw2);
+  }
+  __shared__ EdgeL1 k1s[NEXT ? 16 : 1];
+  __shared__ float c2s[NEXT ? 3 * 64 : 1];
+  EdgeL1 k1;
+  float bias2, sc2, sh2;
+  if constexpr (NEXT) {
+    if (rb == 0) edge_l1_consts(k1s[q], Wc4, b1, s1, t1, q);
+    if (tid < 64) { c2s[tid] = b2 ? b2[tid] : 0.f; c2s[64 + tid] = s2 ? s2[tid] : 1.f; c2s[128 + tid] = s2 ? t2[tid] : 0.f; }
+  } else {
+    edge_l1_consts(k1, Wc4, b1, s1, t1, q);
+    bias2 = b2 ? b2[col] : 0.f; sc2 = s2 ? s2[col] : 1.f; sh2 = s2 ? t2[col] : 0.f;
+  }
+  for (int t = tA; t < tB; ++t) {
+    __syncthreads();
+    if constexpr (NEXT) { k1 = k1s[q]; bias2 = c2s[col]; sc2 = c2s[64 + col]; sh2 = c2s[128 + col]; }
+    const int* cur = ahead[(t - tA) & 1];
+    int* nxt = ahead[(t - tA + 1) & 1];
+    const int n0 = t * npt;
+    const int nn = yl_min(npt, N - n0);
+    const int e0 = cur[128], e1 = cur[128 + nn];
+    int my_b[1], my_e[1];
+    float4 sum[1], fo[1];
+    my_b[0] = cur[128 + yl_min(rb, nn)]; my_e[0] = cur[128 + yl_min(rb + 1, nn)];
+    sum[0] = make_float4(0.f, 0.f, 0.f, 0.f);
+    fo[0] = *reinterpret_cast<const float4*>(f_out + (long)yl_min(n0 + rb, N - 1) * ld_fo + 4 * q);
+    const bool more = t + 1 < tB;
+    int st = 0;
+    if (more) st = start_load(n0 + npt, e1);
+    if (e0 >= e1 && more && tid < 145) nxt[tid] = st;
+    for (int c0 = e0; c0 < e1; c0 += 64) {
+      int di[4], si[4];
+#pragma unroll
+      for (int u = 0; u < 4; ++u) {
+        if (c0 == e0) { di[u] = cur[rb + 16 * u]; si[u] = cur[64 + rb + 16 * u]; }
+        else {
+          const int e = yl_min(c0 + rb + 16 * u, E - 1);
+          di[u] = dst[e]; si[u] = src[e];
+        }
+      }
+      edge_gather_layer1(UV, ld_uv, attr, c0, E, rb, q, di, si, k1, Hs);
+      if (c0 == e0 && more && tid < 145) nxt[tid] = st;
+      __syncthreads();
+      const f32x16 acc2 = edge_mfma_tile(Hs, W2s, wm, wn, l31, lhi);
+      __syncthreads();
+      edge_store_messages(acc2, Hs, wm, lhi, col, bias2, sc2, sh2);
+      __syncthreads();
+      edge_aggregate<1>(Hs, c0, rb, q, nn, my_b, my_e, sum);
+      __syncthreads();
+    }
+    edge_mean_out<1>(f_out, ld_fo, n0, rb, q, nn, my_b, my_e, sum, fo);
+    if constexpr (NEXT) {
+      int lane_t = lane;
+      asm volatile("" : "+v"(lane_t));
+      edge_next_node_side(nx, n0, nn, rb, q, wave, lane_t, fo[0], Hs);
+    }
+  }
 }
 
 typedef __bf16 yl_bf16x8 __attribute__((ext_vector_type(8)));
@@ -775,11 +1036,12 @@
                                    const float* b1, const float* s1, const float* t1, const float* W2, const float* b2,
                                    const float* s2, const float* t2, int64_t C, float* f_out, int64_t ld_fo, int variant,
                                    const PoolRider* rider, int* rode, const EdgeNext* next, int* did_next,
-                                   yolat_stream_t stream) {
+                                   yolat_stream_t stream, int tiles_per_wg) {
   if (rode) *rode = 0;
   if (did_next) *did_next = 0;
   if (E < 0 || N <= 0 || !UV || !Wc4 || !W2 || !row_ptr || !f_out) return YOLAT_E_INVALID;
   if (variant < YOLAT_EDGE_AUTO || variant > YOLAT_EDGE_WS_X6) return YOLAT_E_INVALID;
+  if (tiles_per_wg < 1 || tiles_per_wg > YOLAT_EDGE_MT_MAX) return YOLAT_E_INVALID;
   if (C != 64) return YOLAT_E_UNSUPPORTED;
   if (E == 0) return 0;
   if (!src_csr || !dst_csr || !attr_csr || E >= (1LL << 31) || ld_fo < C || ld_uv < 2 * C) return YOLAT_E_INVALID;
@@ -824,6 +1086,20 @@
     nx = *next;
     if (did_next) *did_next = 1;
   }
+  if (tiles_per_wg > 1 && npt <= 16) {
+    const int wgs = yl_cdiv(tiles, tiles_per_wg);
+    const unsigned mt_grid = (unsigned)wgs + (unsigned)nx.s_tiles + (unsigned)pr.blocks;
+    if (nx.Wp != nullptr)
+      hipLaunchKernelGGL((k_edge_mt_uv_mlp2_mean<true>), dim3(mt_grid), dim3(256), 0, (hipStream_t)stream, UV, (long)ld_uv,
+                         src_csr, dst_csr, attr_csr, row_ptr, (int)N, (int)npt, Wc4, b1, s1, t1, w2, b2, s2, t2, f_out,
+                         (long)ld_fo, (int)E, tiles, tiles_per_wg, wgs, pr, nx);
+    else
+      hipLaunchKernelGGL((k_edge_mt_uv_mlp2_mean<false>), dim3(mt_grid), dim3(256), 0, (hipStream_t)stream, UV, (long)ld_uv,
+                         src_csr, dst_csr, attr_csr, row_ptr, (int)N, (int)npt, Wc4, b1, s1, t1, w2, b2, s2, t2, f_out,
+                         (long)ld_fo, (int)E, tiles, tiles_per_wg, wgs, pr, nx);
+    YL_LAUNCH_CHECK();
+    return 0;
+  }
   const unsigned grid = (unsigned)tiles + (unsigned)nx.s_tiles + (unsigned)pr.blocks;
   if (npt <= 16 && nx.Wp != nullptr)
     hipLaunchKernelGGL((k_edge_uv_mlp2_mean<1, true>), dim3(grid), dim3(256), 0, (hipStream_t)stream, UV, (long)ld_uv,
@@ -849,6 +1125,17 @@
                                                     float* f_out, int64_t ld_fo, int variant, yolat_stream_t stream) {
   return yl_edge_uv_mlp2_mean_eval_impl(UV, ld_uv, src_csr, dst_csr, attr_csr, row_ptr, N, E, Wc4, b1, s1, t1, W2, b2, s2,
                                         t2, C, f_out, ld_fo, variant, nullptr, nullptr, nullptr, nullptr, stream);
+}
+
+extern "C" int yolat_edge_uv_mlp2_mean_eval_mt(const float* UV, int64_t ld_uv, const int32_t* src_csr,
+                                               const int32_t* dst_csr, const float* attr_csr, const int32_t* row_ptr,
+                                               int64_t N, int64_t E, const float* Wc4, const float* b1, const float* s1,
+                                               const float* t1, const float* W2, const float* b2, const float* s2,
+                                               const float* t2, int64_t C, float* f_out, int64_t ld_fo, int tiles_per_wg,
+                                               yolat_stream_t stream) {
+  return yl_edge_uv_mlp2_mean_eval_impl(UV, ld_uv, src_csr, dst_csr, attr_csr, row_ptr, N, E, Wc4, b1, s1, t1, W2, b2, s2,
+                                        t2, C, f_out, ld_fo, YOLAT_EDGE_TILES, nullptr, nullptr, nullptr, nullptr, stream,
+                                        tiles_per_wg);
 }
 
 extern "C" int yolat_edge_uv_mlp2_mean_eval(const float* UV, int64_t ld_uv, const int32_t* src_csr,
diff --git a/yolat_vectorgraphicsrecognition_amd/csrc/forward_eval.hip b/yolat_vectorgraphicsrecognition_amd/csrc/forward_eval.hip
--- a/yolat_vectorgraphicsrecognition_amd/csrc/forward_eval.hip
+++ b/yolat_vectorgraphicsrecognition_amd/csrc/forward_eval.hip
@@ -39,13 +39,14 @@
                         const int64_t* bbox_idx, int64_t E, int64_t N, int64_t P, const Plan& p, int32_t* status,
                         const float* x, int64_t ldx, int64_t Cin, const float* Wuv, const float* uv_bias, const float* Wr,
                         const float* br, const float* Wn, const float* bn, const float* sn, const float* tn, int64_t C,
-                        float* f_out, int64_t ld_fo, float* s_out, int64_t ld_so, bool primed, yolat_stream_t stream) {
+                        float* f_out, int64_t ld_fo, float* s_out, int64_t ld_so, bool primed, yolat_stream_t stream,
+                        int regime) {
   NodeUv a;
   const int rc = yl_build_node_uv(&a, x, ldx, x, ldx, N, Cin, Wuv, uv_bias, Wr, br, Wn, bn, sn, tn, C, p.UV, 2 * C, f_out,
                                   ld_fo, s_out, ld_so);
   if (rc != 0) return rc;
   return yl_graph_prepare_impl(edge, stride_e, stride_c, e_attr, bbox_idx, E, N, P, p.row_ptr, p.perm, p.src, p.dst,
-                               p.attr, p.seg_ptr, p.node_seg, p.work, status, &a, primed, stream);
+                               p.attr, p.seg_ptr, p.node_seg, p.work, status, &a, primed, stream, regime);
 }
 
 #include <stdlib.h>
@@ -119,6 +120,87 @@
   return 0;
 }
 
+#include <atomic>
+#include <chrono>
+#include <mutex>
+#include <string.h>
+namespace {
+constexpr int RG_SLOTS = 64;
+constexpr int RG_STREAMS = 3;
+constexpr uint64_t RG_WINDOW_NS = 1000000ull;
+struct RegimeGauge {
+  std::mutex mu;
+  uint64_t key[RG_SLOTS], seen[RG_SLOTS];
+  bool used[RG_SLOTS];
+};
+RegimeGauge g_gauge{};
+std::atomic<int> g_regime_mode{-1};
+std::atomic<long long> g_regime_counts[2];
+int regime_env_mode() {
+  static const int m = []() {
+    const char* e = getenv("YOLAT_EVAL_REGIME");
+    if (e && !strcmp(e, "latency")) return 1;
+    if (e && !strcmp(e, "throughput")) return 2;
+    return 0;
+  }();
+  return m;
+}
+int regime_streams() {
+  static const int k = []() { const char* e = getenv("YOLAT_EVAL_REGIME_STREAMS"); const int v = e ? atoi(e) : 0;
+                              return v >= 1 ? v : RG_STREAMS; }();
+  return k;
+}
+uint64_t regime_window_ns() {
+  static const uint64_t w = []() { const char* e = getenv("YOLAT_EVAL_REGIME_WINDOW_US"); const long long v = e ? atoll(e) : 0;
+                                   return v >= 1 ? (uint64_t)v * 1000ull : RG_WINDOW_NS; }();
+  return w;
+}
+constexpr int RG_EDGE_MT = 2;
+int regime_edge_mt() {
+  static const int t = []() { const char* e = getenv("YOLAT_EDGE_MT"); const int v = e ? atoi(e) : 0;
+                              return (v >= 1 && v <= YOLAT_EDGE_MT_MAX) ? v : RG_EDGE_MT; }();
+  return t;
+}
+}
+
+extern "C" int yolat_eval_regime_get(void) {
+  const int m = g_regime_mode.load(std::memory_order_relaxed);
+  return m >= 0 ? m : regime_env_mode();
+}
+extern "C" int yolat_eval_regime_set(int mode) {
+  if (mode < 0 || mode > 2) return YOLAT_E_INVALID;
+  g_regime_mode.store(mode, std::memory_order_relaxed);
+  return 0;
+}
+extern "C" int yolat_eval_regime_observe(uint64_t stream_key, uint64_t now_ns) {
+  const uint64_t win = regime_window_ns();
+  int recent = 0;
+  {
+    std::lock_guard<std::mutex> lock(g_gauge.mu);
+    RegimeGauge& t = g_gauge;
+    int slot = -1, spare = -1, oldest = 0;
+    for (int i = 0; i < RG_SLOTS; ++i) {
+      if (t.used[i] && t.key[i] == stream_key) { slot = i; break; }
+      if (!t.used[i]) { if (spare < 0) spare = i; }
+      else if (!t.used[oldest] || t.seen[i] < t.seen[oldest]) oldest = i;
+    }
+    if (slot < 0) slot = spare >= 0 ? spare : oldest;
+    t.used[slot] = true; t.key[slot] = stream_key; t.seen[slot] = now_ns;
+    for (int i = 0; i < RG_SLOTS; ++i)
+      if (t.used[i] && (t.seen[i] >= now_ns ? t.seen[i] - now_ns : now_ns - t.seen[i]) <= win) ++recent;
+  }
+  const int mode = yolat_eval_regime_get();
+  if (mode == 1) return YL_REGIME_LATENCY;
+  if (mode == 2) return YL_REGIME_THROUGHPUT;
+  return recent >= regime_streams() ? YL_REGIME_THROUGHPUT : YL_REGIME_LATENCY;
+}
+extern "C" int yolat_eval_regime_counts(int64_t out[2]) {
+  if (!out) return YOLAT_E_INVALID;
+  out[0] = g_regime_counts[0].load(std::memory_order_relaxed);
+  out[1] = g_regime_counts[1].load(std::memory_order_relaxed);
+  return 0;
+}
+
 static int cls1_x6(const float* Z, long ZW, long P, uint16_t* Zs, const uint16_t* Wp, const float* shift, long H1,
                    float* c1, yolat_stream_t stream) {
   YL_TRY(yolat_split_bf16x3_packed(Z, ZW, P, ZW, nullptr, Zs, stream));
@@ -177,6 +259,11 @@
   Plan p = carve(m, N, E, P, workspace);
   if (p.bytes > workspace_bytes) return YOLAT_E_INVALID;
   if (g != nullptr) YL_TRY(yl_adopt_graph(g, E, &p));
+  const int regime = yolat_eval_regime_observe(
+      (uint64_t)(uintptr_t)stream,
+      (uint64_t)std::chrono::duration_cast<std::chrono::nanoseconds>(std::chrono::steady_clock::now().time_since_epoch()).count());
+  g_regime_counts[regime].fetch_add(1, std::memory_order_relaxed);
+  const int edge_mt = regime == YL_REGIME_THROUGHPUT ? regime_edge_mt() : 1;
   const long C = m->C, F = m->F, D = C * m->n_blocks_out, ZW = 2 * (F + D);
   const int lo = m->n_blocks - m->n_blocks_out;
 
@@ -204,11 +291,11 @@
              16.0 * E + 12.0 * E + 32.0 * E + 12.0 * N + 4.0 * (2.0 * N * cv0.Cin + 4.0 * N * C),
              prep_node_uv(edge, stride_e, stride_c, e_attr, bbox_idx, E, N, P, p, status, x, ldx, cv0.Cin,
                           fold0 ? cv0.Wuvf : cv0.Wuv, fold0 ? cv0.uvb : nullptr, cv0.Wr, cv0.br, cv0.Wn, cv0.bn, cv0.sn,
-                          cv0.tn, C, f0, ld0, s0, ld0, primed, stream));
+                          cv0.tn, C, f0, ld0, s0, ld0, primed, stream, regime));
   } else if (g == nullptr) {
   YL_STAGE("graph_prep[csr+attr+segments]", 0, 16.0 * E + 12.0 * E + 32.0 * E + 12.0 * N,
            yl_graph_prepare_impl(edge, stride_e, stride_c, e_attr, bbox_idx, E, N, P, p.row_ptr, p.perm, p.src,
-                                 p.dst, p.attr, p.seg_ptr, p.node_seg, p.work, status, nullptr, primed, stream));
+                                 p.dst, p.attr, p.seg_ptr, p.node_seg, p.work, status, nullptr, primed, stream, regime));
   }
 
   static const bool riders_on = []() { const char* v = getenv("YOLAT_POOL_RIDERS"); return !(v && v[0] == '0'); }();
@@ -276,10 +363,11 @@
                    fold ? yl_edge_uv_mlp2_mean_eval_impl(uv_l, 2 * C, p.src, p.dst, p.attr, p.row_ptr, N, E, cv.Wc4f,
                                                          nullptr, nullptr, nullptr, cv.W2, nullptr, cv.s2, cv.t2f, C,
                                                          f_out, ld_out, YOLAT_EDGE_AUTO, rd, &rode,
-                                                         nx.Wp ? &nx : nullptr, &did_next, stream)
+                                                         nx.Wp ? &nx : nullptr, &did_next, stream, edge_mt)
                         : yl_edge_uv_mlp2_mean_eval_impl(uv_l, 2 * C, p.src, p.dst, p.attr, p.row_ptr, N, E, cv.Wc4,
                                                          cv.b1, cv.s1, cv.t1, cv.W2, cv.b2, cv.s2, cv.t2, C, f_out,
-                                                         ld_out, YOLAT_EDGE_AUTO, rd, &rode, nullptr, nullptr, stream));
+                                                         ld_out, YOLAT_EDGE_AUTO, rd, &rode, nullptr, nullptr, stream,
+                                                         edge_mt));
           if (rode) pool_done |= ride_a.parts;
           next_done = did_next != 0;
           uv_next = nx.UV;
diff --git a/yolat_vectorgraphicsrecognition_amd/csrc/graph.hip b/yolat_vectorgraphicsrecognition_amd/csrc/graph.hip
--- a/yolat_vectorgraphicsrecognition_amd/csrc/graph.hip
+++ b/yolat_vectorgraphicsrecognition_amd/csrc/graph.hip
@@ -608,9 +608,10 @@
 }
 
 #define PS_PLAN_ROWS 100
+#define PS_PLAN_ROWS_TP 250
 #define PS_PLAN_EDGES (PS_CAP / 2)
 #define PS_PLAN_GRID 250
-static int prep_small_rows(int64_t N, int64_t E, int64_t other_blocks) {
+static int prep_small_rows(int64_t N, int64_t E, int64_t other_blocks, int regime) {
   static const bool on = []() { const char* e = getenv("YOLAT_PREP_SMALL"); return !(e && e[0] == '0'); }();
   static const int forced = []() { const char* e = getenv("YOLAT_PREP_R"); const int r = e ? atoi(e) : 0;
                                    return (r >= 1 && r <= PS_RMAX) ? r : 0; }();
@@ -618,7 +619,8 @@
   if (forced) return forced;
   int64_t r_edges = E > 0 ? (int64_t)PS_PLAN_EDGES * N / E : PS_RMAX;
   if (r_edges < 1) r_edges = 1;
-  int64_t R = PS_PLAN_ROWS;
+  int64_t R = regime == YL_REGIME_THROUGHPUT ? PS_PLAN_ROWS_TP : PS_PLAN_ROWS;
+  if (R > PS_RMAX) R = PS_RMAX;
   if (R > r_edges) R = r_edges;
   if (R > N) R = N;
   if ((N + R - 1) / R + other_blocks > PS_PLAN_GRID) {
@@ -630,11 +632,17 @@
   return (int)R;
 }
 
-extern "C" int yolat_graph_prepare_plan(int64_t N, int64_t E, int64_t other_wgs, int32_t* rows, int32_t* csr_wgs) {
-  const int R = (other_wgs < 0) ? 0 : prep_small_rows(N, E, other_wgs);
+extern "C" int yolat_graph_prepare_plan_regime(int64_t N, int64_t E, int64_t other_wgs, int regime, int32_t* rows,
+                                               int32_t* csr_wgs) {
+  const bool ok = other_wgs >= 0 && (regime == YL_REGIME_LATENCY || regime == YL_REGIME_THROUGHPUT);
+  const int R = ok ? prep_small_rows(N, E, other_wgs, regime) : 0;
   if (rows) *rows = R;
   if (csr_wgs) *csr_wgs = R > 0 ? (int32_t)((N + R - 1) / R) : 0;
   return R > 0 ? 1 : 0;
+}
+
+extern "C" int yolat_graph_prepare_plan(int64_t N, int64_t E, int64_t other_wgs, int32_t* rows, int32_t* csr_wgs) {
+  return yolat_graph_prepare_plan_regime(N, E, other_wgs, YL_REGIME_LATENCY, rows, csr_wgs);
 }
 
 extern "C" size_t yolat_graph_work_elems(int64_t N, int64_t E) {
@@ -645,7 +653,7 @@
                               const int64_t* bbox_idx, int64_t E, int64_t N, int64_t P, int32_t* row_ptr,
                               int32_t* perm, int32_t* src_csr, int32_t* dst_csr, float* attr_csr, int32_t* seg_ptr,
                               int32_t* node_seg, int32_t* work, int32_t* status, const NodeUv* extra, bool primed,
-                              yolat_stream_t stream) {
+                              yolat_stream_t stream, int regime) {
   if (N <= 0 || E < 0 || N >= (1LL << 31) - 8192 || E >= (1LL << 31) - 256) return YOLAT_E_INVALID;
   if (!row_ptr || !work || !status) return YOLAT_E_INVALID;
   if (E > 0 && (!edge || !e_attr || !perm || !src_csr || !dst_csr || !attr_csr)) return YOLAT_E_INVALID;
@@ -664,7 +672,7 @@
   int* items = rank + E;
   const int node_blocks = extra ? yl_cdiv(extra->N, 8 * PS_NW * PS_NODE_ITERS) : 0;
   const int seg_blocks = bbox_idx ? yl_cdiv(N + 1, PS_T) : 0;
-  const int Rs = (extra == nullptr || yl_node3_smallk_shape_ok(*extra)) ? prep_small_rows(N, E, node_blocks + seg_blocks) : 0;
+  const int Rs = (extra == nullptr || yl_node3_smallk_shape_ok(*extra)) ? prep_small_rows(N, E, node_blocks + seg_blocks, regime) : 0;
   if (Rs > 0) {
     PrepSmall g;
     g.edge = edge; g.se = (long)stride_e; g.sc = (long)stride_c; g.attr = reinterpret_cast<const float4*>(e_attr);
diff --git a/yolat_vectorgraphicsrecognition_amd/ops.py b/yolat_vectorgraphicsrecognition_amd/ops.py
--- a/yolat_vectorgraphicsrecognition_amd/ops.py
+++ b/yolat_vectorgraphicsrecognition_amd/ops.py
@@ -659,6 +659,18 @@
     return f_out
 
 
+def edge_uv_mlp2_mean_eval_mt(UV, g, wc4, b1, pro1, W2, b2, pro2, f_out, tiles_per_wg=1):
+    s1, t1 = pro1 if pro1 is not None else (None, None)
+    s2, t2 = pro2 if pro2 is not None else (None, None)
+    check(lib.yolat_edge_uv_mlp2_mean_eval_mt(_f(UV, "UV"), _ld(UV), g.src.data_ptr(), g.dst.data_ptr(),
+                                              g.attr.data_ptr(), g.row_ptr.data_ptr(), g.N, g.E, _f(wc4),
+                                              _f(b1, "b1", True), _f(s1, "s1", True), _f(t1, "t1", True), _f(W2),
+                                              _f(b2, "b2", True), _f(s2, "s2", True), _f(t2, "t2", True),
+                                              W2.shape[0], _f(f_out), _ld(f_out), int(tiles_per_wg), _stream()),
+          "yolat_edge_uv_mlp2_mean_eval_mt")
+    return f_out
+
+
 def edge_mlp2_eval(x, g, W1, b1, pro1, W2, b2, pro2, H2):
     N, Cin = x.shape
     C = W1.shape[0]
```
